# UVA-Computer-Vision-Lab/midvision-probe

Hardware: AMD Instinct MI355X
Metric: images/sec feature-extract+probe-step, ViT-B/16 224^2 (higher is better)
Workload: dtype f16x2 (compensated fp16 pairs of activations and frozen weights, two f16 MFMA products per contraction, fp32 accumulate, feature error as bf16x3; attention: Q.K^T the same two products over compensated pairs, P.V fp16 probabilities x (fp16 + bf16) V; probe, fp32 residual/LN/softmax/loss as in bf16x3

## Files before the change

### include/mvp_hip.h

```cpp
#ifndef MVP_HIP_H
#define MVP_HIP_H

#include <stdint.h>

#ifdef __cplusplus
extern "C" {
#endif

#define MVP_OK 0
#define MVP_EINVAL (-1)
#define MVP_ELAUNCH (-2)
#define MVP_ENODEV (-3)

#define MVP_PREC_BF16 1
#define MVP_PREC_BF16X3 3
#define MVP_PREC_F16X2 2

#define MVP_ACT_NONE 0
#define MVP_ACT_GELU 1
#define MVP_ACT_RELU 2
#define MVP_ACT_QUICK_GELU 3
#define MVP_ACT_GELU_TANH 4

typedef uint16_t mvp_bf16;

typedef struct {
  int abi_version;
  int device_count;
  int gfx950;
  int cu_count;
  char arch[64];
} mvp_info_t;
#define MVP_ABI_VERSION 8
int mvp_get_info(mvp_info_t* out);
const char* mvp_strerror(int code);
int mvp_sizeof(const char* struct_name);

typedef struct {
  const float* src;
  mvp_bf16* hi;
  mvp_bf16* lo;
  int64_t n;
} mvp_split_bf16_args;
int mvp_split_bf16(const mvp_split_bf16_args*, void* stream);

typedef struct {
  const float* images;
  mvp_bf16* out_hi;
  mvp_bf16* out_lo;
  int B, C, H, W;
  int P;
  int gh, gw;
  int pad_top, pad_left;
} mvp_patch_gather_args;
int mvp_patch_gather(const mvp_patch_gather_args*, void* stream);
typedef struct mvp_patch_gather_ld_args mvp_patch_gather_ld_args;
struct mvp_patch_gather_ld_args {
  mvp_patch_gather_args g;
  int ldk;
};
int mvp_patch_gather_ld(const mvp_patch_gather_ld_args*, void* stream);

typedef struct {
  const mvp_bf16* a_hi; const mvp_bf16* a_lo;
  const mvp_bf16* w_hi; const mvp_bf16* w_lo;
  const float* bias;
  const float* residual;
  float* out_f32;
  mvp_bf16* out_hi;
  mvp_bf16* out_lo;
  int M, N, K;
  int lda, ldw, ldr, ldo, ldob;
  int act;
  int precision;
  int row_group, row_group_stride, row_group_off, res_row_mod;
  int conv, cH, cW, cC, cHo, cWo, ckh, ckw, cstride, cpad, cup;
  const mvp_bf16* zero_page;
  const uint8_t* relu_mask; uint8_t* out_mask; int ldm; int mask_mode;
  const float* residual2;
  int act_after_res;
  int splitk; void* splitk_ws; int64_t splitk_ws_bytes;
  const mvp_bf16* residual_hi; const mvp_bf16* residual_lo;
  int tile_policy;
  int pair_layout;
  int out_pair_layout;
  int out_f16_col0;
} mvp_gemm_args;
#define MVP_TILES_ALONE 0
#define MVP_TILES_SHARED 1
#define MVP_TILES_NO_PP 2
#define MVP_TILES_NO_UNI 4
#define MVP_PAIR_SEPARATE 0
#define MVP_PAIR_A_ILV32 1
#define MVP_PAIR_W_ILV32 2
#define MVP_PAIR_ILV32 3
int mvp_gemm_bias_act_res(const mvp_gemm_args*, void* stream);
int mvp_gemm_pp(const mvp_gemm_args*, void* stream);
int64_t mvp_gemm_splitk_workspace_bytes(int M, int N, int splits);
#define MVP_GEMM_ROUTE_PP 1
#define MVP_GEMM_ROUTE_TILE 2
#define MVP_GEMM_ROUTE_SPLITK 3
#define MVP_GEMM_ROUTE_CONV 4
typedef struct mvp_gemm_route_t mvp_gemm_route_t;
struct mvp_gemm_route_t {
  int family;
  int bm, bn, bk;
  int split;
  int nstage, nw, wnw;
};
int mvp_gemm_route(const mvp_gemm_args*, mvp_gemm_route_t* out);
typedef struct mvp_gemm_scaled_args mvp_gemm_scaled_args;
struct mvp_gemm_scaled_args {
  mvp_gemm_args gemm;
  const float* col_scale;
};
int mvp_gemm_scaled(const mvp_gemm_scaled_args*, void* stream);

typedef struct {
  const float* x; const float* gamma; const float* beta;
  mvp_bf16* out_hi; mvp_bf16* out_lo;
  float* out_f32;
  int M, C;
  float eps;
  int out_layout;
  int out_f16;
} mvp_layernorm_args;
int mvp_layernorm_fwd(const mvp_layernorm_args*, void* stream);

typedef struct {
  const mvp_bf16* qkv_hi; const mvp_bf16* qkv_lo;
  mvp_bf16* out_hi; mvp_bf16* out_lo;
  int B, N, H;
  int ld_qkv, ld_out;
  float scale;
  int precision;
  int out_layout;
  int v_format;
  int out_f16;
} mvp_attention_args;
#define MVP_ATT_V_BF16_PAIR 0
#define MVP_ATT_V_F16 1
#define MVP_ATT_V_F16_QK_F16 2
int mvp_attention_fwd(const mvp_attention_args*, void* stream);

typedef struct mvp_attention_bias_args mvp_attention_bias_args;
struct mvp_attention_bias_args {
  mvp_attention_args att;
  const float* bias;
  int64_t bias_head_stride;
  int ld_bias;
};
int mvp_attention_bias_fwd(const mvp_attention_bias_args*, void* stream);

typedef struct mvp_rope2d_qkv_args mvp_rope2d_qkv_args;
struct mvp_rope2d_qkv_args {
  const float* qkv;
  mvp_bf16* out_hi; mvp_bf16* out_lo;
  const float* cos_tab; const float* sin_tab;
  int M, N, H;
  int n_prefix, gh, gw;
  int tab_rows;
  int ld_in, ld_out;
  int precision, v_format;
};
int mvp_rope2d_qkv(const mvp_rope2d_qkv_args*, void* stream);

typedef struct mvp_gather_rows_args mvp_gather_rows_args;
struct mvp_gather_rows_args {
  const mvp_bf16* in_hi; const mvp_bf16* in_lo;
  mvp_bf16* out_hi; mvp_bf16* out_lo;
  const int* idx;
  int rows, rows_in, cols;
  int ld_in, ld_out;
};
int mvp_gather_rows(const mvp_gather_rows_args*, void* stream);

typedef struct mvp_relpos_terms_args mvp_relpos_terms_args;
struct mvp_relpos_terms_args {
  const float* qkv;
  mvp_bf16* out_hi; mvp_bf16* out_lo;
  float* rel;
  const float* rh; const float* rw;
  int64_t rel_bh_stride;
  int M, N, H;
  int Qh, Qw, Kh, Kw;
  int ld_in, ld_out, ld_rel;
  int precision, v_format;
};
int mvp_relpos_terms(const mvp_relpos_terms_args*, void* stream);

typedef struct mvp_attention_relpos_args mvp_attention_relpos_args;
struct mvp_attention_relpos_args {
  mvp_attention_args att;
  const float* rel;
  int64_t rel_bh_stride;
  int ld_rel;
  int Kh, Kw;
};
int mvp_attention_relpos_fwd(const mvp_attention_relpos_args*, void* stream);

typedef struct {
  const float* cls; const float* pos0; float* x; int B, N, C;
} mvp_cls_rows_args;
int mvp_cls_rows(const mvp_cls_rows_args*, void* stream);
typedef struct mvp_prefix_rows_args mvp_prefix_rows_args;
struct mvp_prefix_rows_args {
  const float* cls; const float* pos0; const float* reg; float* x; int B, N, C, R;
};
int mvp_prefix_rows(const mvp_prefix_rows_args*, void* stream);

typedef struct {
  const float* x;
  const float* gamma; const float* beta;
  float* running_mean; float* running_var;
  float* stats;
  float* nchw;
  mvp_bf16* tok_hi; mvp_bf16* tok_lo; int ld_tok; int col_off;
  mvp_bf16* tokT_hi; mvp_bf16* tokT_lo; int ldT;
  void* workspace; int64_t workspace_bytes;
  int B, N, C, hw;
  float eps, momentum;
  int mode;
  float* cls_out;
  int64_t* num_batches_tracked;
  int defer_running;
  int groups;
  int64_t stats_gstride, nchw_gstride, tok_gstride, cls_gstride;
} mvp_bn_tokens_args;
int64_t mvp_bn_tokens_workspace_bytes(int M, int C);
int mvp_bn_tokens_to_nchw_fwd(const mvp_bn_tokens_args*, void* stream);

typedef struct {
  const float* stats;
  float* running_mean; float* running_var;
  int64_t* num_batches_tracked;
  int C; float momentum;
} mvp_bn_running_update_args;
int mvp_bn_running_update(const mvp_bn_running_update_args*, void* stream);
#define MVP_BN_RUNNING_MAX 8
int mvp_bn_running_update_n(const mvp_bn_running_update_args* items, int n, void* stream);

typedef struct {
  const float* nchw;
  mvp_bf16* tok_hi; mvp_bf16* tok_lo; int ld_tok; int col_off;
  mvp_bf16* tokT_hi; mvp_bf16* tokT_lo; int ldT;
  int B, C, hw;
} mvp_pack_nchw_args;
int mvp_pack_nchw_tokens(const mvp_pack_nchw_args*, void* stream);

#define MVP_RESIZE_NEAREST 0
#define MVP_RESIZE_BILINEAR 1
#define MVP_RESIZE_BICUBIC 2
typedef struct {
  const float* src; float* dst;
  int planes, Hi, Wi, Ho, Wo;
  int mode; int align_corners;
  int channels_last; int C;
  float scale_h, scale_w;
} mvp_resize_args;
int mvp_resize_fwd(const mvp_resize_args*, void* stream);
int mvp_resize_bwd(const mvp_resize_args*, void* stream);
int mvp_resize_aa_fwd(const mvp_resize_args*, void* stream);

typedef struct {
  const float* logits; float* depth; float* inv_sum;
  const float* grad_depth; float* grad_logits;
  int64_t P; int K;
  float min_depth, max_depth;
  int kind;
} mvp_depth_predict_args;
int mvp_depth_predict_fwd(const mvp_depth_predict_args*, void* stream);
int mvp_depth_predict_bwd(const mvp_depth_predict_args*, void* stream);

typedef struct {
  const float* pred; float* target; float* loss; float* grad_pred;
  void* workspace; int64_t workspace_bytes;
  int B; int64_t HW;
  float w_sig, w_grad, max_depth, eps, sigma;
} mvp_depth_loss_args;
int64_t mvp_depth_loss_workspace_bytes(int B, int64_t HW);
int mvp_depth_loss_fwd_bwd(const mvp_depth_loss_args*, void* stream);

typedef struct {
  const float* pred; const float* gt; const uint8_t* mask;
  float* loss; float* grad_pred;
  void* workspace; int64_t workspace_bytes;
  int B; int Cp; int64_t HW;
  float eps;
} mvp_angular_loss_args;
int mvp_angular_loss_fwd_bwd(const mvp_angular_loss_args*, void* stream);

typedef struct {
  const float* x; float* out; int M, N, ld;
  int accumulate;
  void* workspace; int64_t workspace_bytes;
} mvp_colsum_args;
int64_t mvp_colsum_workspace_bytes(int M, int N);
int mvp_colsum(const mvp_colsum_args*, void* stream);

typedef struct {
  float* param; const float* grad; float* exp_avg; float* exp_avg_sq;
  const float* hyper; int64_t n;
  float beta1, beta2, eps, weight_decay, grad_scale;
  float lr, bias_c1, bias_c2;
} mvp_adamw_args;
int mvp_adamw_step(const mvp_adamw_args*, void* stream);

typedef struct {
  const float* src_feat; const float* tgt_feat;
  const float* kp_xy;
  int64_t* out_xy; float* out_val;
  float* workspace; int64_t workspace_bytes;
  int C, h, w, K;
  float* heat_out;
} mvp_corr_argmax_args;
int64_t mvp_corr_workspace_bytes(int C, int h, int w, int K);
int mvp_corr_argmax(const mvp_corr_argmax_args*, void* stream);
typedef struct {
  const float* x; int64_t* out_xy; int K, h, w, max_value;
} mvp_argmax_2d_args;
int mvp_argmax_2d(const mvp_argmax_2d_args*, void* stream);

typedef struct mvp_knn_ratio_args mvp_knn_ratio_args;
struct mvp_knn_ratio_args {
  const float* src_feat; const float* tgt_feat;
  const uint8_t* src_valid; const uint8_t* tgt_valid;
  int32_t* nn_idx;
  float* dist;
  float* weight;
  int32_t* n_valid;
  void* workspace; int64_t workspace_bytes;
  int C, N0, N1;
};
int64_t mvp_knn_workspace_bytes(int C, int N0, int N1);
int mvp_knn_ratio(const mvp_knn_ratio_args*, void* stream);

#define MVP_BN_ACT_MAX_C 8
#define MVP_BN_ACT_NONE 0
#define MVP_BN_ACT_SIGMOID 1
#define MVP_BN_ACT_TANH 2
#define MVP_BN_ACT_WORKSPACE_BYTES 98304
typedef struct mvp_bn_act_args mvp_bn_act_args;
struct mvp_bn_act_args {
  const float* x; float* y;
  const float* gamma; const float* beta;
  float* running_mean; float* running_var; int64_t* num_batches_tracked;
  float* stats;
  const float* grad_y; float* grad_x; float* grad_gamma; float* grad_beta;
  void* workspace; int64_t workspace_bytes;
  int B; int64_t HW; int C; int ld;
  int64_t n;
  float eps, momentum;
  int act, training, accumulate;
};
int mvp_bn_act_fwd(const mvp_bn_act_args*, void* stream);
int mvp_bn_act_bwd(const mvp_bn_act_args*, void* stream);

#define MVP_BCE_WORKSPACE_BYTES 8192
typedef struct mvp_bce_loss_args mvp_bce_loss_args;
struct mvp_bce_loss_args {
  const float* pred; const float* target; float* loss; float* grad_pred;
  void* workspace; int64_t workspace_bytes;
  int64_t N;
};
int mvp_bce_loss_fwd_bwd(const mvp_bce_loss_args*, void* stream);

typedef struct mvp_binary_counts_args mvp_binary_counts_args;
struct mvp_binary_counts_args {
  const float* pred; const float* gt; int64_t* counts;
  int G; int64_t n;
  float threshold;
};
int mvp_binary_counts(const mvp_binary_counts_args*, void* stream);

typedef struct {
  const float* w; mvp_bf16* out_hi; mvp_bf16* out_lo;
  int Cout, Cin, kh, kw, mode;
} mvp_conv_weight_pack_args;
int mvp_conv_weight_pack(const mvp_conv_weight_pack_args*, void* stream);

typedef struct {
  const float* src; float* dst_f32; mvp_bf16* dst_hi; mvp_bf16* dst_lo;
  int B, H, W, C, f; int backward;
} mvp_upsample_cl_args;
int mvp_upsample_nearest_cl(const mvp_upsample_cl_args*, void* stream);

typedef struct {
  const float* g; mvp_bf16* out_hi; mvp_bf16* out_lo;
  int B, H, W, C, f;
} mvp_upconv_boxsum_args;
int mvp_upconv3_grad_boxsum(const mvp_upconv_boxsum_args*, void* stream);

typedef struct {
  const float* t; const float* bias; float* out_f32; mvp_bf16* out_hi; mvp_bf16* out_lo; uint8_t* out_mask;
  int B, H, W, C, f, act;
} mvp_upconv_gather_args;
int mvp_upconv3_fwd_gather(const mvp_upconv_gather_args*, void* stream);

typedef struct {
  const mvp_bf16* g_hi; const mvp_bf16* g_lo; const mvp_bf16* x_hi; const mvp_bf16* x_lo;
  float* partial; float* dw; const mvp_bf16* zero_page;
  int64_t M; int Cout, Cin, ldg, ldx;
  int H, W, Ho, Wo, kh, kw, stride, pad, up;
  int splits, accumulate, precision;
} mvp_gemm_tn_args;
typedef struct {
  const float* pred; const float* gt; float* out; float* scale_shift;
  void* workspace; int64_t workspace_bytes; int B; int64_t HW; int scale_invariant;
} mvp_depth_metrics_args;
typedef struct {
  const float* pred; const float* gt; float* out;
  void* workspace; int64_t workspace_bytes; int B; int Cp; int64_t HW; float t1, t2, t3;
} mvp_snorm_metrics_args;
int64_t mvp_metrics_workspace_bytes(int B);
int mvp_depth_metrics(const mvp_depth_metrics_args*, void* stream);
int mvp_snorm_metrics(const mvp_snorm_metrics_args*, void* stream);
typedef struct {
  const float* x; const float* scale_shift; const float* grad_out; float* out;
  int B; int64_t HW; float lo, hi; int clamp; int backward;
} mvp_scale_shift_args;
int mvp_scale_shift(const mvp_scale_shift_args*, void* stream);

typedef struct {
  const float* pred; const float* gt; const int32_t* seg; const float* scale_shift;
  double* level_sums; double* seg_sums;
  void* workspace; int64_t workspace_bytes;
  int B, H, W, Cp, num_levels, num_ids;
  float t1, t2, t3;
} mvp_metrics_breakdown_args;
int64_t mvp_metrics_breakdown_workspace_bytes(int B, int num_levels, int num_ids);
int mvp_metrics_breakdown(const mvp_metrics_breakdown_args*, void* stream);

typedef struct {
  const float* l0; float* depth; float* inv_sum; uint8_t* gate;
  const float* grad_depth; float* grad_l0;
  int B, h, w, K, f;
  float min_depth, max_depth;
} mvp_linear_bins_args;
int mvp_linear_bins_fwd(const mvp_linear_bins_args*, void* stream);
int mvp_linear_bins_bwd(const mvp_linear_bins_args*, void* stream);

typedef struct {
  const float* src; mvp_bf16* out_hi; mvp_bf16* out_lo;
  int B, C, H, W, Ho, Wo, kh, kw, stride, pad, ldk;
} mvp_im2col_args;
int mvp_im2col_nchw(const mvp_im2col_args*, void* stream);

typedef struct {
  const float* src; float* dst_f32; mvp_bf16* dst_hi; mvp_bf16* dst_lo;
  int B, H, W, C, Ho, Wo, k, stride, pad;
} mvp_maxpool_cl_args;
int mvp_maxpool_cl(const mvp_maxpool_cl_args*, void* stream);

typedef struct {
  const float* images; const mvp_bf16* w_hi; const mvp_bf16* w_lo; const float* bias;
  float* out_f32; mvp_bf16* out_hi; mvp_bf16* out_lo;
  int B, H, W, precision;
} mvp_stem_args;
int mvp_stem7x7_pool(const mvp_stem_args*, void* stream);

typedef struct {
  const float* src; const uint8_t* mask; float* dst_f32; mvp_bf16* dst_hi; mvp_bf16* dst_lo;
  int64_t M; int N, lds, ldm, ldo;
  uint8_t* relu_mask_out;
} mvp_mask_split_args;
int mvp_mask_split(const mvp_mask_split_args*, void* stream);

int64_t mvp_gemm_tn_workspace_bytes(int Cout, int Cin, int kh, int kw, int splits);
int mvp_gemm_tn_conv(const mvp_gemm_tn_args*, void* stream);

#ifdef __cplusplus
}
#endif
#endif
```

### midvision-probe_amd/csrc/head.hip

```cpp
#include "mvp_common.h"

namespace {

__device__ __forceinline__ float bin_value(int k, int K, float lo, float hi) {
  const float step = (hi - lo) / (float)(K - 1);
  return (k < K / 2) ? lo + step * (float)k : hi - step * (float)(K - 1 - k);
}

__device__ __forceinline__ void bil_taps(float scale, int o, int in, int& i0, int& i1, float& w0, float& w1) {
  const float s = fmaxf(scale * ((float)o + 0.5f) - 0.5f, 0.f);
  i0 = min((int)s, in - 1);
  i1 = i0 + (i0 < in - 1 ? 1 : 0);
  w1 = s - (float)i0;
  w0 = 1.f - w1;
}

__global__ __launch_bounds__(256) void linear_bins_fwd_kernel(const mvp_linear_bins_args p) {
  const int lane = threadIdx.x & 63;
  const int Ho = p.h * p.f, Wo = p.w * p.f;
  const int64_t px = (int64_t)blockIdx.x * 4 + (threadIdx.x >> 6);
  if (px >= (int64_t)p.B * Ho * Wo) return;
  const int x = (int)(px % Wo);
  const int64_t r = px / Wo;
  const int y = (int)(r % Ho);
  const int64_t b = r / Ho;
  const float sc = 1.0f / (float)p.f;
  int y0, y1, x0, x1;
  float wy0, wy1, wx0, wx1;
  bil_taps(sc, y, p.h, y0, y1, wy0, wy1);
  bil_taps(sc, x, p.w, x0, x1, wx0, wx1);
  const float* base = p.l0 + b * p.h * p.w * p.K;
  const float* r00 = base + ((size_t)y0 * p.w + x0) * p.K;
  const float* r01 = base + ((size_t)y0 * p.w + x1) * p.K;
  const float* r10 = base + ((size_t)y1 * p.w + x0) * p.K;
  const float* r11 = base + ((size_t)y1 * p.w + x1) * p.K;
  const float w00 = wy0 * wx0, w01 = wy0 * wx1, w10 = wy1 * wx0, w11 = wy1 * wx1;
  float s = 0.f, d = 0.f;
  uint8_t* gate = p.gate + px * (p.K >> 3);
  for (int k = lane * 4; k < p.K; k += 256) {
    const float4 a = *(const float4*)(r00 + k), bq = *(const float4*)(r01 + k), c = *(const float4*)(r10 + k), e = *(const float4*)(r11 + k);
    float l[4] = {wy0 * (wx0 * a.x + wx1 * bq.x) + wy1 * (wx0 * c.x + wx1 * e.x), wy0 * (wx0 * a.y + wx1 * bq.y) + wy1 * (wx0 * c.y + wx1 * e.y),
                  wy0 * (wx0 * a.z + wx1 * bq.z) + wy1 * (wx0 * c.z + wx1 * e.z), wy0 * (wx0 * a.w + wx1 * bq.w) + wy1 * (wx0 * c.w + wx1 * e.w)};
    (void)w00; (void)w01; (void)w10; (void)w11;
    unsigned nib = 0;
#pragma unroll
    for (int q = 0; q < 4; ++q) {
      nib |= (l[q] > 0.f ? 1u : 0u) << q;
      const float pq = fmaxf(l[q], 0.f) + 0.1f;
      s += pq;
      d += pq * bin_value(k + q, p.K, p.min_depth, p.max_depth);
    }
    const unsigned other = __shfl_xor(nib, 1, 64);
    if ((lane & 1) == 0) gate[k >> 3] = (uint8_t)(nib | (other << 4));
  }
  s = wave_sum(s);
  d = wave_sum(d);
  if (lane == 0) {
    const float inv = 1.0f / s;
    p.depth[px] = d * inv;
    p.inv_sum[px] = inv;
  }
}

__global__ __launch_bounds__(256) void linear_bins_bwd_kernel(const mvp_linear_bins_args p) {
  const int lane = threadIdx.x & 63;
  const int Ho = p.h * p.f, Wo = p.w * p.f;
  const int64_t tok = (int64_t)blockIdx.x * 4 + (threadIdx.x >> 6);
  if (tok >= (int64_t)p.B * p.h * p.w) return;
  const int tx = (int)(tok % p.w);
  const int64_t r = tok / p.w;
  const int ty = (int)(r % p.h);
  const int64_t b = r / p.h;
  const float sc = 1.0f / (float)p.f;
  const float ff = (float)p.f;
  int ylo = max(0, (int)floorf(ff * ((float)ty - 0.5f) - 0.5f) - 1), yhi = min(Ho - 1, (int)ceilf(ff * ((float)ty + 1.5f) - 0.5f) + 1);
  int xlo = max(0, (int)floorf(ff * ((float)tx - 0.5f) - 0.5f) - 1), xhi = min(Wo - 1, (int)ceilf(ff * ((float)tx + 1.5f) - 0.5f) + 1);
  if (ty == 0) ylo = 0;
  if (ty == p.h - 1) yhi = Ho - 1;
  if (tx == 0) xlo = 0;
  if (tx == p.w - 1) xhi = Wo - 1;
  const int KB = p.K >> 3;
  for (int k = lane * 4; k < p.K; k += 256) {
    float s1[4] = {0.f, 0.f, 0.f, 0.f}, s2[4] = {0.f, 0.f, 0.f, 0.f};
    for (int oy = ylo; oy <= yhi; ++oy) {
      int i0, i1; float w0, w1;
      bil_taps(sc, oy, p.h, i0, i1, w0, w1);
      const float wy = (i0 == ty ? w0 : 0.f) + (i1 == ty ? w1 : 0.f);
      if (wy == 0.f) continue;
      for (int ox = xlo; ox <= xhi; ++ox) {
        bil_taps(sc, ox, p.w, i0, i1, w0, w1);
        const float wx = (i0 == tx ? w0 : 0.f) + (i1 == tx ? w1 : 0.f);
        if (wx == 0.f) continue;
        const int64_t px = (b * Ho + oy) * Wo + ox;
        const float a = wy * wx * p.grad_depth[px] * p.inv_sum[px];
        const float bb = a * p.depth[px];
        const unsigned byte = p.gate[px * KB + (k >> 3)];
        const unsigned nib = (lane & 1) ? (byte >> 4) : (byte & 15u);
#pragma unroll
        for (int q = 0; q < 4; ++q) {
          const float m = (float)((nib >> q) & 1u);
          s1[q] += a * m;
          s2[q] += bb * m;
        }
      }
    }
    float4 o;
    o.x = bin_value(k, p.K, p.min_depth, p.max_depth) * s1[0] - s2[0];
    o.y = bin_value(k + 1, p.K, p.min_depth, p.max_depth) * s1[1] - s2[1];
    o.z = bin_value(k + 2, p.K, p.min_depth, p.max_depth) * s1[2] - s2[2];
    o.w = bin_value(k + 3, p.K, p.min_depth, p.max_depth) * s1[3] - s2[3];
    *(float4*)(p.grad_l0 + tok * p.K + k) = o;
  }
}


__device__ __forceinline__ int bil_cell(float scale, int o, int in) {
  const float s = scale * ((float)o + 0.5f) - 0.5f;
  return (s < 0.f) ? -1 : min((int)s, in - 1);
}

__global__ __launch_bounds__(256) void linear_bins_fwd_cells(const mvp_linear_bins_args p) {
  __shared__ __attribute__((aligned(16))) uint8_t gate_s[4][16][32];
  __shared__ float dep_s[4][16], inv_s[4][16];
  __shared__ int px_s[4][16];
  const int lane = threadIdx.x & 63, wave = threadIdx.x >> 6;
  const int Ho = p.h * p.f, Wo = p.w * p.f;
  const int cells_x = p.w + 1, cells_y = p.h + 1;
  const int64_t cell = (int64_t)blockIdx.x * 4 + wave;
  if (cell >= (int64_t)p.B * cells_y * cells_x) return;
  const int cx = (int)(cell % cells_x) - 1;
  const int64_t r = cell / cells_x;
  const int cy = (int)(r % cells_y) - 1;
  const int64_t b = r / cells_y;
  const float sc = 1.0f / (float)p.f, ff = (float)p.f;
  const int r0 = max(cy, 0), r1 = min(r0 + 1, p.h - 1), c0 = max(cx, 0), c1 = min(c0 + 1, p.w - 1);
  const float* base = p.l0 + b * p.h * p.w * 256;
  const int k = lane * 4;
  const float4 a = *(const float4*)(base + ((size_t)r0 * p.w + c0) * 256 + k);
  const float4 bq = *(const float4*)(base + ((size_t)r0 * p.w + c1) * 256 + k);
  const float4 c = *(const float4*)(base + ((size_t)r1 * p.w + c0) * 256 + k);
  const float4 e = *(const float4*)(base + ((size_t)r1 * p.w + c1) * 256 + k);
  float bins[4];
#pragma unroll
  for (int q = 0; q < 4; ++q) bins[q] = bin_value(k + q, 256, p.min_depth, p.max_depth);
  const int ylo = max(0, (int)floorf(ff * ((float)cy + 0.5f) - 0.5f) - 1), yhi = min(Ho - 1, (int)ceilf(ff * ((float)cy + 1.5f) - 0.5f) + 1);
  const int xlo = max(0, (int)floorf(ff * ((float)cx + 0.5f) - 0.5f) - 1), xhi = min(Wo - 1, (int)ceilf(ff * ((float)cx + 1.5f) - 0.5f) + 1);
  int npix = 0;
  for (int y = ylo; y <= yhi; ++y) {
    if (bil_cell(sc, y, p.h) != cy) continue;
    int y0, y1; float wy0, wy1;
    bil_taps(sc, y, p.h, y0, y1, wy0, wy1);
    for (int x = xlo; x <= xhi; ++x) {
      if (bil_cell(sc, x, p.w) != cx) continue;
      int x0, x1; float wx0, wx1;
      bil_taps(sc, x, p.w, x0, x1, wx0, wx1);
      const float l[4] = {wy0 * (wx0 * a.x + wx1 * bq.x) + wy1 * (wx0 * c.x + wx1 * e.x), wy0 * (wx0 * a.y + wx1 * bq.y) + wy1 * (wx0 * c.y + wx1 * e.y),
                          wy0 * (wx0 * a.z + wx1 * bq.z) + wy1 * (wx0 * c.z + wx1 * e.z), wy0 * (wx0 * a.w + wx1 * bq.w) + wy1 * (wx0 * c.w + wx1 * e.w)};
      float s = 0.f, d = 0.f;
      unsigned nib = 0;
#pragma unroll
      for (int q = 0; q < 4; ++q) {
        nib |= (l[q] > 0.f ? 1u : 0u) << q;
        const float pq = fmaxf(l[q], 0.f) + 0.1f;
        s += pq;
        d += pq * bins[q];
      }
      const unsigned other = __shfl_xor(nib, 1, 64);
      if ((lane & 1) == 0) gate_s[wave][npix][lane >> 1] = (uint8_t)(nib | (other << 4));
      s = wave_sum(s);
      d = wave_sum(d);
      if (lane == 0) {
        const float inv = 1.0f / s;
        dep_s[wave][npix] = d * inv;
        inv_s[wave][npix] = inv;
        px_s[wave][npix] = (int)(((int)b * Ho + y) * Wo + x);
      }
      ++npix;
    }
  }
  __builtin_amdgcn_fence(__ATOMIC_RELEASE, "wavefront");
  __builtin_amdgcn_wave_barrier();
  __builtin_amdgcn_fence(__ATOMIC_ACQUIRE, "wavefront");
  if (lane < npix) {
    const int px = px_s[wave][lane];
    p.depth[px] = dep_s[wave][lane];
    p.inv_sum[px] = inv_s[wave][lane];
  }
  if (lane < 2 * npix) {
    const int pi = lane >> 1, half = lane & 1;
    *(u32x4_t*)(p.gate + (size_t)px_s[wave][pi] * 32 + half * 16) = *(const u32x4_t*)&gate_s[wave][pi][half * 16];
  }
}

__global__ __launch_bounds__(256) void linear_bins_bwd_fast(const mvp_linear_bins_args p) {
  const int lane = threadIdx.x & 63;
  const int Ho = p.h * p.f, Wo = p.w * p.f;
  const int64_t tok = (int64_t)blockIdx.x * 4 + (threadIdx.x >> 6);
  if (tok >= (int64_t)p.B * p.h * p.w) return;
  const int tx = (int)(tok % p.w);
  const int64_t r = tok / p.w;
  const int ty = (int)(r % p.h);
  const int64_t b = r / p.h;
  const float sc = 1.0f / (float)p.f, ff = (float)p.f;
  int ylo = max(0, (int)floorf(ff * ((float)ty - 0.5f) - 0.5f) - 1), yhi = min(Ho - 1, (int)ceilf(ff * ((float)ty + 1.5f) - 0.5f) + 1);
  int xlo = max(0, (int)floorf(ff * ((float)tx - 0.5f) - 0.5f) - 1), xhi = min(Wo - 1, (int)ceilf(ff * ((float)tx + 1.5f) - 0.5f) + 1);
  if (ty == 0) ylo = 0;
  if (ty == p.h - 1) yhi = Ho - 1;
  if (tx == 0) xlo = 0;
  if (tx == p.w - 1) xhi = Wo - 1;
  const int ny = yhi - ylo + 1, nx = xhi - xlo + 1, ncand = ny * nx;
  const int k = lane * 4;
  float s1[4] = {0.f, 0.f, 0.f, 0.f}, s2[4] = {0.f, 0.f, 0.f, 0.f};
  for (int c0 = 0; c0 < ncand; c0 += 64) {
    const int ci = c0 + lane;
    float a_l = 0.f, bb_l = 0.f;
    int px_l = 0;
    if (ci < ncand) {
      const int oy = ylo + ci / nx, ox = xlo + ci % nx;
      int i0, i1; float w0, w1;
      bil_taps(sc, oy, p.h, i0, i1, w0, w1);
      const float wy = (i0 == ty ? w0 : 0.f) + (i1 == ty ? w1 : 0.f);
      bil_taps(sc, ox, p.w, i0, i1, w0, w1);
      const float wx = (i0 == tx ? w0 : 0.f) + (i1 == tx ? w1 : 0.f);
      if (wy != 0.f && wx != 0.f) {
        px_l = (int)(((int)b * Ho + oy) * Wo + ox);
        a_l = wy * wx * p.grad_depth[px_l] * p.inv_sum[px_l];
        bb_l = a_l * p.depth[px_l];
      }
    }
    unsigned long long live = __ballot(a_l != 0.f || bb_l != 0.f);
    while (live) {
      int idx[8];
      unsigned byte[8];
      int n = 0;
#pragma unroll
      for (int u = 0; u < 8; ++u) {
        idx[u] = -1;
        if (live) {
          idx[u] = __builtin_ctzll(live);
          live &= live - 1;
          n = u + 1;
        }
      }
#pragma unroll
      for (int u = 0; u < 8; ++u)
        if (u < n) byte[u] = p.gate[(size_t)__shfl(px_l, idx[u], 64) * 32 + (lane >> 1)];
#pragma unroll
      for (int u = 0; u < 8; ++u) {
        if (u < n) {
          const float av = __shfl(a_l, idx[u], 64), bv = __shfl(bb_l, idx[u], 64);
          const unsigned nib = (lane & 1) ? (byte[u] >> 4) : (byte[u] & 15u);
#pragma unroll
          for (int q = 0; q < 4; ++q) {
            const float m = (float)((nib >> q) & 1u);
            s1[q] += av * m;
            s2[q] += bv * m;
          }
        }
      }
    }
  }
  float4 o;
  o.x = bin_value(k, 256, p.min_depth, p.max_depth) * s1[0] - s2[0];
  o.y = bin_value(k + 1, 256, p.min_depth, p.max_depth) * s1[1] - s2[1];
  o.z = bin_value(k + 2, 256, p.min_depth, p.max_depth) * s1[2] - s2[2];
  o.w = bin_value(k + 3, 256, p.min_depth, p.max_depth) * s1[3] - s2[3];
  *(float4*)(p.grad_l0 + tok * 256 + k) = o;
}

}

extern "C" int mvp_linear_bins_fwd(const mvp_linear_bins_args* a, void* stream) {
  if (!a || !a->l0 || !a->depth || !a->inv_sum || !a->gate) return MVP_EINVAL;
  if (a->B <= 0 || a->h <= 0 || a->w <= 0 || a->f < 1 || a->K < 8 || (a->K & 7)) return MVP_EINVAL;
  const int64_t P = (int64_t)a->B * a->h * a->f * a->w * a->f;
  static const bool generic = getenv("MVP_BINS_GENERIC") != nullptr;
  if (!generic && a->K == 256 && a->f <= 4 && P < ((int64_t)1 << 31)) {
    const int64_t cells = (int64_t)a->B * (a->h + 1) * (a->w + 1);
    hipLaunchKernelGGL(linear_bins_fwd_cells, dim3((unsigned)((cells + 3) / 4)), dim3(256), 0, (hipStream_t)stream, *a);
  } else {
    hipLaunchKernelGGL(linear_bins_fwd_kernel, dim3((unsigned)((P + 3) / 4)), dim3(256), 0, (hipStream_t)stream, *a);
  }
  MVP_LAUNCH_CHECK();
  return MVP_OK;
}

extern "C" int mvp_linear_bins_bwd(const mvp_linear_bins_args* a, void* stream) {
  if (!a || !a->grad_depth || !a->grad_l0 || !a->depth || !a->inv_sum || !a->gate) return MVP_EINVAL;
  if (a->B <= 0 || a->h <= 0 || a->w <= 0 || a->f < 1 || a->K < 8 || (a->K & 7)) return MVP_EINVAL;
  const int64_t T = (int64_t)a->B * a->h * a->w;
  if (a->K == 256 && a->f <= 4 && T * a->f * a->f < ((int64_t)1 << 31))
    hipLaunchKernelGGL(linear_bins_bwd_fast, dim3((unsigned)((T + 3) / 4)), dim3(256), 0, (hipStream_t)stream, *a);
  else
    hipLaunchKernelGGL(linear_bins_bwd_kernel, dim3((unsigned)((T + 3) / 4)), dim3(256), 0, (hipStream_t)stream, *a);
  MVP_LAUNCH_CHECK();
  return MVP_OK;
}
```

### midvision-probe_amd/csrc/info.hip

```cpp
#include <string.h>

#include "mvp_common.h"

extern "C" int mvp_get_info(mvp_info_t* out) {
  if (!out) return MVP_EINVAL;
  memset(out, 0, sizeof(*out));
  out->abi_version = MVP_ABI_VERSION;
  int n = 0;
  if (hipGetDeviceCount(&n) != hipSuccess) n = 0;
  out->device_count = n;
  if (n > 0) {
    hipDeviceProp_t prop;
    if (hipGetDeviceProperties(&prop, 0) == hipSuccess) {
      strncpy(out->arch, prop.gcnArchName, sizeof(out->arch) - 1);
      out->cu_count = prop.multiProcessorCount;
      out->gfx950 = strncmp(prop.gcnArchName, "gfx950", 6) == 0;
    }
  }
  return MVP_OK;
}

extern "C" int mvp_sizeof(const char* name) {
  if (!name) return -1;
#define MVP_SZ(T) if (strcmp(name, #T) == 0) return (int)sizeof(T);
  MVP_SZ(mvp_info_t) MVP_SZ(mvp_split_bf16_args) MVP_SZ(mvp_patch_gather_args) MVP_SZ(mvp_gemm_args) MVP_SZ(mvp_layernorm_args)
  MVP_SZ(mvp_attention_args) MVP_SZ(mvp_cls_rows_args) MVP_SZ(mvp_bn_tokens_args) MVP_SZ(mvp_pack_nchw_args) MVP_SZ(mvp_resize_args)
  MVP_SZ(mvp_depth_predict_args) MVP_SZ(mvp_depth_loss_args) MVP_SZ(mvp_angular_loss_args) MVP_SZ(mvp_colsum_args) MVP_SZ(mvp_adamw_args)
  MVP_SZ(mvp_corr_argmax_args) MVP_SZ(mvp_conv_weight_pack_args) MVP_SZ(mvp_upsample_cl_args) MVP_SZ(mvp_upconv_boxsum_args) MVP_SZ(mvp_upconv_gather_args) MVP_SZ(mvp_gemm_tn_args)
  MVP_SZ(mvp_depth_metrics_args) MVP_SZ(mvp_snorm_metrics_args) MVP_SZ(mvp_linear_bins_args) MVP_SZ(mvp_im2col_args)
  MVP_SZ(mvp_maxpool_cl_args) MVP_SZ(mvp_mask_split_args) MVP_SZ(mvp_metrics_breakdown_args) MVP_SZ(mvp_argmax_2d_args) MVP_SZ(mvp_scale_shift_args) MVP_SZ(mvp_stem_args) MVP_SZ(mvp_bn_running_update_args)
  MVP_SZ(mvp_gemm_scaled_args) MVP_SZ(mvp_patch_gather_ld_args) MVP_SZ(mvp_prefix_rows_args) MVP_SZ(mvp_gemm_route_t) MVP_SZ(mvp_rope2d_qkv_args) MVP_SZ(mvp_attention_bias_args)
  MVP_SZ(mvp_gather_rows_args) MVP_SZ(mvp_relpos_terms_args) MVP_SZ(mvp_attention_relpos_args) MVP_SZ(mvp_knn_ratio_args)
  MVP_SZ(mvp_bn_act_args) MVP_SZ(mvp_bce_loss_args) MVP_SZ(mvp_binary_counts_args)
#undef MVP_SZ
  return -1;
}

extern "C" const char* mvp_strerror(int code) {
  switch (code) {
    case MVP_OK: return "ok";
    case MVP_EINVAL: return "invalid argument (shape, alignment or NULL pointer)";
    case MVP_ELAUNCH: return "HIP kernel launch failed";
    case MVP_ENODEV: return "no gfx950 device";
    default: return "unknown error";
  }
}
```

### midvision-probe_amd/csrc/optim.hip

```cpp
#include "mvp_common.h"

namespace {

__global__ __launch_bounds__(256) void adamw_kernel(const mvp_adamw_args p) {
  const float lr = p.hyper ? p.hyper[0] : p.lr, bc1 = p.hyper ? p.hyper[1] : p.bias_c1, bc2 = p.hyper ? p.hyper[2] : p.bias_c2;
  const float step_size = lr / bc1;
  const float rbc2 = 1.0f / sqrtf(bc2);
  const float decay = 1.0f - lr * p.weight_decay;
  const int64_t n4 = p.n >> 2;
  for (int64_t i = (int64_t)blockIdx.x * 256 + threadIdx.x; i < n4; i += (int64_t)gridDim.x * 256) {
    float4 w = ((float4*)p.param)[i];
    const float4 g4 = ((const float4*)p.grad)[i];
    float4 m = ((float4*)p.exp_avg)[i];
    float4 v = ((float4*)p.exp_avg_sq)[i];
    float* wp = (float*)&w; const float* gp = (const float*)&g4; float* mp = (float*)&m; float* vp = (float*)&v;
#pragma unroll
    for (int e = 0; e < 4; ++e) {
      const float g = gp[e] * p.grad_scale;
      wp[e] *= decay;
      mp[e] = p.beta1 * mp[e] + (1.f - p.beta1) * g;
      vp[e] = p.beta2 * vp[e] + (1.f - p.beta2) * g * g;
      wp[e] -= step_size * mp[e] / (sqrtf(vp[e]) * rbc2 + p.eps);
    }
    ((float4*)p.param)[i] = w;
    ((float4*)p.exp_avg)[i] = m;
    ((float4*)p.exp_avg_sq)[i] = v;
  }
  if (blockIdx.x == 0 && threadIdx.x < (p.n & 3)) {
    const int64_t i = (n4 << 2) + threadIdx.x;
    const float g = p.grad[i] * p.grad_scale;
    float w = p.param[i] * decay;
    const float m = p.beta1 * p.exp_avg[i] + (1.f - p.beta1) * g;
    const float v = p.beta2 * p.exp_avg_sq[i] + (1.f - p.beta2) * g * g;
    w -= step_size * m / (sqrtf(v) * rbc2 + p.eps);
    p.param[i] = w; p.exp_avg[i] = m; p.exp_avg_sq[i] = v;
  }
}

}

extern "C" int mvp_adamw_step(const mvp_adamw_args* a, void* stream) {
  if (!a || !a->param || !a->grad || !a->exp_avg || !a->exp_avg_sq || a->n <= 0) return MVP_EINVAL;
  if (!a->hyper && !(a->bias_c1 > 0.f && a->bias_c2 > 0.f)) return MVP_EINVAL;
  if (((uintptr_t)a->param | (uintptr_t)a->grad | (uintptr_t)a->exp_avg | (uintptr_t)a->exp_avg_sq) & 15) return MVP_EINVAL;
  int64_t g = ((a->n >> 2) + 255) / 256;
  if (g < 1) g = 1;
  if (g > 2048) g = 2048;
  hipLaunchKernelGGL(adamw_kernel, dim3((unsigned)g), dim3(256), 0, (hipStream_t)stream, *a);
  MVP_LAUNCH_CHECK();
  return MVP_OK;
}
```

### midvision-probe_amd/csrc/probe.hip

```cpp
#include "mvp_common.h"

namespace {

__device__ __forceinline__ float bin_value(int k, int K, float lo, float hi) {
  const float step = (hi - lo) / (float)(K - 1);
  return (k < K / 2) ? lo + step * (float)k : hi - step * (float)(K - 1 - k);
}

__global__ __launch_bounds__(256) void depth_bins_fwd(const mvp_depth_predict_args p) {
  const int lane = threadIdx.x & 63;
  const int64_t px = (int64_t)blockIdx.x * 4 + (threadIdx.x >> 6);
  if (px >= p.P) return;
  const float* l = p.logits + px * p.K;
  float s = 0.f, d = 0.f;
  for (int k = lane * 4; k < p.K; k += 256) {
    const float4 v = *(const float4*)(l + k);
    const float a = fmaxf(v.x, 0.f) + 0.1f, b = fmaxf(v.y, 0.f) + 0.1f, c = fmaxf(v.z, 0.f) + 0.1f, e = fmaxf(v.w, 0.f) + 0.1f;
    s += (a + b) + (c + e);
    d += a * bin_value(k, p.K, p.min_depth, p.max_depth) + b * bin_value(k + 1, p.K, p.min_depth, p.max_depth) +
         c * bin_value(k + 2, p.K, p.min_depth, p.max_depth) + e * bin_value(k + 3, p.K, p.min_depth, p.max_depth);
  }
  s = wave_sum(s);
  d = wave_sum(d);
  if (lane == 0) {
    const float inv = 1.0f / s;
    p.depth[px] = d * inv;
    if (p.inv_sum) p.inv_sum[px] = inv;
  }
}

__global__ __launch_bounds__(256) void depth_bins_bwd(const mvp_depth_predict_args p) {
  const int lane = threadIdx.x & 63;
  const int64_t px = (int64_t)blockIdx.x * 4 + (threadIdx.x >> 6);
  if (px >= p.P) return;
  const float* l = p.logits + px * p.K;
  float* g = p.grad_logits + px * p.K;
  const float depth = p.depth[px];
  const float gs = p.grad_depth[px] * p.inv_sum[px];
  for (int k = lane * 4; k < p.K; k += 256) {
    const float4 v = *(const float4*)(l + k);
    float4 o;
    o.x = v.x > 0.f ? gs * (bin_value(k, p.K, p.min_depth, p.max_depth) - depth) : 0.f;
    o.y = v.y > 0.f ? gs * (bin_value(k + 1, p.K, p.min_depth, p.max_depth) - depth) : 0.f;
    o.z = v.z > 0.f ? gs * (bin_value(k + 2, p.K, p.min_depth, p.max_depth) - depth) : 0.f;
    o.w = v.w > 0.f ? gs * (bin_value(k + 3, p.K, p.min_depth, p.max_depth) - depth) : 0.f;
    *(float4*)(g + k) = o;
  }
}

__global__ __launch_bounds__(256) void depth_sigmoid_fwd(const mvp_depth_predict_args p) {
  for (int64_t i = (int64_t)blockIdx.x * 256 + threadIdx.x; i < p.P; i += (int64_t)gridDim.x * 256) {
    const float s = 1.0f / (1.0f + expf(-p.logits[i]));
    p.depth[i] = p.min_depth + s * (p.max_depth - p.min_depth);
  }
}

__global__ __launch_bounds__(256) void depth_sigmoid_bwd(const mvp_depth_predict_args p) {
  for (int64_t i = (int64_t)blockIdx.x * 256 + threadIdx.x; i < p.P; i += (int64_t)gridDim.x * 256) {
    const float s = 1.0f / (1.0f + expf(-p.logits[i]));
    p.grad_logits[i] = p.grad_depth[i] * (p.max_depth - p.min_depth) * s * (1.0f - s);
  }
}

constexpr int CS_CHUNK = 64;

__host__ __device__ inline int cs_chunk_rows(int M) {
  const int r = (M + 255) / 256;
  return r < CS_CHUNK ? CS_CHUNK : ((r + 3) & ~3);
}

__global__ __launch_bounds__(256) void colsum_partial_kernel(const mvp_colsum_args p, float* part, int chunk) {
  __shared__ float red[4][64];
  const int c = blockIdx.x * 64 + (threadIdx.x & 63);
  const int rg = threadIdx.x >> 6;
  const int r0 = blockIdx.y * chunk, r1 = min(p.M, r0 + chunk);
  float s = 0.f;
  if (c < p.N) {
    float s0 = 0.f, s1 = 0.f, s2 = 0.f, s3 = 0.f;
    int r = r0 + rg;
    for (; r + 12 < r1; r += 16) {
      s0 += p.x[(size_t)r * p.ld + c];
      s1 += p.x[(size_t)(r + 4) * p.ld + c];
      s2 += p.x[(size_t)(r + 8) * p.ld + c];
      s3 += p.x[(size_t)(r + 12) * p.ld + c];
    }
    for (; r < r1; r += 4) s0 += p.x[(size_t)r * p.ld + c];
    s = (s0 + s1) + (s2 + s3);
  }
  red[rg][threadIdx.x & 63] = s;
  __syncthreads();
  if (rg == 0 && c < p.N)
    part[(size_t)blockIdx.y * p.N + c] = (red[0][threadIdx.x] + red[1][threadIdx.x]) + (red[2][threadIdx.x] + red[3][threadIdx.x]);
}

__global__ __launch_bounds__(256) void colsum_final_kernel(const mvp_colsum_args p, const float* part, int nchunk) {
  __shared__ float red[4][64];
  const int lc = threadIdx.x & 63, rg = threadIdx.x >> 6;
  const int c = blockIdx.x * 64 + lc;
  float s0 = 0.f, s1 = 0.f, s2 = 0.f, s3 = 0.f;
  if (c < p.N) {
    int k = rg;
    for (; k + 12 < nchunk; k += 16) {
      s0 += part[(size_t)k * p.N + c];
      s1 += part[(size_t)(k + 4) * p.N + c];
      s2 += part[(size_t)(k + 8) * p.N + c];
      s3 += part[(size_t)(k + 12) * p.N + c];
    }
    for (; k < nchunk; k += 4) s0 += part[(size_t)k * p.N + c];
  }
  red[rg][lc] = (s0 + s1) + (s2 + s3);
  __syncthreads();
  if (rg == 0 && c < p.N) {
    const float s = (red[0][lc] + red[1][lc]) + (red[2][lc] + red[3][lc]);
    p.out[c] = p.accumulate ? p.out[c] + s : s;
  }
}

inline int grid_for(int64_t work) {
  int64_t g = (work + 255) / 256;
  return (int)(g < 1 ? 1 : (g > 4096 ? 4096 : g));
}

}

extern "C" int mvp_depth_predict_fwd(const mvp_depth_predict_args* a, void* stream) {
  if (!a || !a->logits || !a->depth || a->P <= 0 || a->K <= 0) return MVP_EINVAL;
  hipStream_t s = (hipStream_t)stream;
  if (a->kind == 0) {
    if ((a->K & 3) || a->K < 2) return MVP_EINVAL;
    hipLaunchKernelGGL(depth_bins_fwd, dim3((unsigned)((a->P + 3) / 4)), dim3(256), 0, s, *a);
  } else {
    if (a->K != 1) return MVP_EINVAL;
    hipLaunchKernelGGL(depth_sigmoid_fwd, dim3(grid_for(a->P)), dim3(256), 0, s, *a);
  }
  MVP_LAUNCH_CHECK();
  return MVP_OK;
}

extern "C" int mvp_depth_predict_bwd(const mvp_depth_predict_args* a, void* stream) {
  if (!a || !a->logits || !a->grad_depth || !a->grad_logits || a->P <= 0 || a->K <= 0) return MVP_EINVAL;
  hipStream_t s = (hipStream_t)stream;
  if (a->kind == 0) {
    if ((a->K & 3) || !a->depth || !a->inv_sum) return MVP_EINVAL;
    hipLaunchKernelGGL(depth_bins_bwd, dim3((unsigned)((a->P + 3) / 4)), dim3(256), 0, s, *a);
  } else {
    if (a->K != 1) return MVP_EINVAL;
    hipLaunchKernelGGL(depth_sigmoid_bwd, dim3(grid_for(a->P)), dim3(256), 0, s, *a);
  }
  MVP_LAUNCH_CHECK();
  return MVP_OK;
}

extern "C" int64_t mvp_colsum_workspace_bytes(int M, int N) {
  const int chunk = cs_chunk_rows(M);
  return (int64_t)((M + chunk - 1) / chunk) * N * 4;
}

extern "C" int mvp_colsum(const mvp_colsum_args* a, void* stream) {
  if (!a || !a->x || !a->out || !a->workspace || a->M <= 0 || a->N <= 0 || a->ld < a->N) return MVP_EINVAL;
  if (a->workspace_bytes < mvp_colsum_workspace_bytes(a->M, a->N)) return MVP_EINVAL;
  const int chunk = cs_chunk_rows(a->M);
  const int nchunk = (a->M + chunk - 1) / chunk;
  hipStream_t s = (hipStream_t)stream;
  hipLaunchKernelGGL(colsum_partial_kernel, dim3((a->N + 63) / 64, nchunk), dim3(256), 0, s, *a, (float*)a->workspace, chunk);
  hipLaunchKernelGGL(colsum_final_kernel, dim3((a->N + 63) / 64), dim3(256), 0, s, *a, (const float*)a->workspace, nchunk);
  MVP_LAUNCH_CHECK();
  return MVP_OK;
}

namespace {
__global__ __launch_bounds__(256) void mask_split_kernel(const mvp_mask_split_args p) {
  const int64_t total = (int64_t)p.M * p.ldo;
  for (int64_t i = (int64_t)blockIdx.x * 256 + threadIdx.x; i < total; i += (int64_t)gridDim.x * 256) {
    const int c = (int)(i % p.ldo);
    const int64_t r = i / p.ldo;
    float v = 0.f;
    if (c < p.N) {
      v = p.src[r * p.lds + c];
      if (p.mask && !p.mask[r * p.ldm + c]) v = 0.f;
      if (p.relu_mask_out) { const bool on = v > 0.f; v = on ? v : 0.f; p.relu_mask_out[r * p.ldm + c] = on; }
      if (p.dst_f32) p.dst_f32[r * p.lds + c] = v;
    }
    uint16_t h, l;
    split_bf16(v, h, l);
    if (p.dst_hi) p.dst_hi[i] = h;
    if (p.dst_lo) p.dst_lo[i] = l;
  }
}

__global__ __launch_bounds__(256) void mask_split_vec4_kernel(const mvp_mask_split_args p) {
  const int q = p.ldo >> 2;
  const int64_t total = (int64_t)p.M * q;
  for (int64_t i = (int64_t)blockIdx.x * 256 + threadIdx.x; i < total; i += (int64_t)gridDim.x * 256) {
    const int64_t r = i / q;
    const int c = (int)(i - r * q) << 2;
    float4 v = make_float4(0.f, 0.f, 0.f, 0.f);
    if (c < p.N) {
      v = *(const float4*)(p.src + r * p.lds + c);
      if (p.mask) {
        const uint32_t m = *(const uint32_t*)(p.mask + r * p.ldm + c);
        if (!(m & 0xffu)) v.x = 0.f;
        if (!(m & 0xff00u)) v.y = 0.f;
        if (!(m & 0xff0000u)) v.z = 0.f;
        if (!(m & 0xff000000u)) v.w = 0.f;
      }
      if (p.relu_mask_out) {
        const uint32_t m = (v.x > 0.f ? 1u : 0u) | (v.y > 0.f ? 0x100u : 0u) | (v.z > 0.f ? 0x10000u : 0u) | (v.w > 0.f ? 0x1000000u : 0u);
        v.x = fmaxf(v.x, 0.f); v.y = fmaxf(v.y, 0.f); v.z = fmaxf(v.z, 0.f); v.w = fmaxf(v.w, 0.f);
        *(uint32_t*)(p.relu_mask_out + r * p.ldm + c) = m;
      }
      if (p.dst_f32) *(float4*)(p.dst_f32 + r * p.lds + c) = v;
    }
    uint32_t h01, l01, h23, l23;
    split2_bf16(v.x, v.y, h01, l01);
    split2_bf16(v.z, v.w, h23, l23);
    const int64_t o = r * p.ldo + c;
    if (p.dst_hi) *(u32x2_t*)(p.dst_hi + o) = u32x2_t{h01, h23};
    if (p.dst_lo) *(u32x2_t*)(p.dst_lo + o) = u32x2_t{l01, l23};
  }
}
}

extern "C" int mvp_mask_split(const mvp_mask_split_args* a, void* stream) {
  if (!a || !a->src || a->M <= 0 || a->N <= 0 || a->ldo < a->N || a->lds < a->N) return MVP_EINVAL;
  const bool vec = !((a->N | a->ldo | a->lds) & 3) && ((!a->mask && !a->relu_mask_out) || !(a->ldm & 3)) &&
                   !(((uintptr_t)a->src | (uintptr_t)a->dst_f32) & 15) && !(((uintptr_t)a->dst_hi | (uintptr_t)a->dst_lo) & 7) &&
                   !(((uintptr_t)a->mask | (uintptr_t)a->relu_mask_out) & 3);
  int64_t g = ((int64_t)a->M * (vec ? a->ldo >> 2 : a->ldo) + 255) / 256;
  if (g > 16384) g = 16384;
  if (vec)
    hipLaunchKernelGGL(mask_split_vec4_kernel, dim3((unsigned)g), dim3(256), 0, (hipStream_t)stream, *a);
  else
    hipLaunchKernelGGL(mask_split_kernel, dim3((unsigned)g), dim3(256), 0, (hipStream_t)stream, *a);
  MVP_LAUNCH_CHECK();
  return MVP_OK;
}
```

### midvision-probe_amd/mvp/functional.py

```python
from __future__ import annotations

from typing import List, Optional, Sequence, Tuple

import torch

from . import lib, ops, pipeline
from .lib import PREC_BF16, PREC_BF16X3
from .vit import PackedFeatures, lookup_pack

_MODES = {"nearest": lib.RESIZE_NEAREST, "bilinear": lib.RESIZE_BILINEAR, "bicubic": lib.RESIZE_BICUBIC}


def _need_cuda(t: torch.Tensor, what: str):
    if not t.is_cuda:
        raise lib.MvpError(f"{what}: the HIP path needs device tensors (there is no CPU fallback)")


class _Interpolate(torch.autograd.Function):
    @staticmethod
    def forward(ctx, x, Ho, Wo, mode, align, sh, sw):
        _need_cuda(x, "interpolate")
        x = x.contiguous().float()
        B, C, Hi, Wi = x.shape
        y = torch.empty(B, C, Ho, Wo, dtype=torch.float32, device=x.device)
        ops.resize(x, y, B * C, Hi, Wi, Ho, Wo, mode, align_corners=align, scale_h=sh, scale_w=sw)
        ctx.cfg = (B, C, Hi, Wi, Ho, Wo, mode, align, sh, sw)
        return y

    @staticmethod
    def backward(ctx, gy):
        B, C, Hi, Wi, Ho, Wo, mode, align, sh, sw = ctx.cfg
        gy = gy.contiguous().float()
        gx = torch.empty(B, C, Hi, Wi, dtype=torch.float32, device=gy.device)
        ops.resize(gy, gx, B * C, Hi, Wi, Ho, Wo, mode, align_corners=align, scale_h=sh, scale_w=sw, backward=True)
        return gx, None, None, None, None, None, None


def interpolate(x: torch.Tensor, size=None, scale_factor=None, mode: str = "nearest", align_corners: Optional[bool] = None) -> torch.Tensor:
    if mode not in _MODES:
        raise NotImplementedError(f"interpolate mode {mode!r}")
    Hi, Wi = x.shape[-2:]
    sh = sw = 0.0
    if size is not None:
        Ho, Wo = (size, size) if isinstance(size, int) else tuple(int(s) for s in size)
    else:
        sf = (scale_factor, scale_factor) if not isinstance(scale_factor, (tuple, list)) else scale_factor
        sh, sw = float(sf[0]), float(sf[1])
        Ho, Wo = int(Hi * sh), int(Wi * sw)
    return _Interpolate.apply(x, Ho, Wo, _MODES[mode], bool(align_corners), sh, sw)


def resize_antialias(x: torch.Tensor, size) -> torch.Tensor:
    _need_cuda(x, "resize_antialias")
    if x.requires_grad:
        raise lib.MvpError("resize_antialias is forward-only (input side of the frozen backbone)")
    x = x.contiguous().float()
    B, C, Hi, Wi = x.shape
    Ho, Wo = (size, size) if isinstance(size, int) else tuple(int(v) for v in size)
    y = torch.empty(B, C, Ho, Wo, dtype=torch.float32, device=x.device)
    a = lib.ResizeArgs(lib.ptr(x), lib.ptr(y), B * C, Hi, Wi, Ho, Wo, lib.RESIZE_BILINEAR, 0, 0, 0, 0.0, 0.0)
    lib.call("mvp_resize_aa_fwd", a)
    return y


def pack_features(feats: Sequence[torch.Tensor], precision: int) -> PackedFeatures:
    pack = lookup_pack(feats)
    if pack is not None and pack.precision == precision:
        return pack
    B, _, h, w = feats[0].shape
    for f in feats:
        _need_cuda(f, "probe features")
        if f.shape[0] != B or f.shape[-2:] != (h, w):
            raise lib.MvpError("linear head: all feature maps must share batch and resolution (reference quirk Q7)")
    Ctot = sum(int(f.shape[1]) for f in feats)
    pack = PackedFeatures(B, h, w, Ctot, precision, feats[0].device)
    off = 0
    for f in feats:
        C = int(f.shape[1])
        ops.pack_nchw_tokens(f.contiguous().float(), B, C, h * w, tok=pack.tok, ld_tok=pack.Cpad, col_off=off)
        off += C
    return pack


def _grad_dst(param, shape):
    from .optim import grad_destination

    d = grad_destination(param) if param is not None else None
    return d.view(shape) if d is not None and d.numel() == int(torch.Size(shape).numel()) else None


def _head_weight_grad(gl0: torch.Tensor, K: int, pack: PackedFeatures, pr: int, dst: Optional[torch.Tensor] = None) -> torch.Tensor:
    from . import conv
    dev = gl0.device
    Kg = (K + 127) // 128 * 128
    if Kg != K:
        gpad = gl0.new_zeros(pack.M, Kg)
        gpad[:, :K] = gl0
        gl0 = gpad
    gp = ops.split_bf16(gl0, pr)
    dW = dst if (dst is not None and pack.Cpad == pack.Ctot and tuple(dst.shape) == (K, pack.Cpad)) else torch.empty(K, pack.Cpad, dtype=torch.float32, device=dev)
    geo = dict(B=pack.B, H=pack.h, W=pack.w, C=pack.Cpad, Ho=pack.h, Wo=pack.w, kh=1, kw=1, stride=1, pad=0, up=0)
    conv.conv_dw(gp, Kg, pack.tok, pack.Cpad, geo, K, dW, precision=pr)
    return dW[:, :pack.Ctot]


class _LinearHeadK1(torch.autograd.Function):

    @staticmethod
    def forward(ctx, weight, bias, pack: PackedFeatures, precision: int):
        K, Ctot = weight.shape[0], pack.Ctot
        K4 = (K + 3) // 4 * 4
        dev = weight.device
        w2 = weight.detach().reshape(K, Ctot).float()
        b1 = bias.detach().float()
        if K4 != K or pack.Cpad != Ctot:
            wpad = w2.new_zeros(K4, pack.Cpad)
            wpad[:K, :Ctot] = w2
            w2 = wpad
            b1 = torch.cat([b1, b1.new_zeros(K4 - K)], 0)
        wp = ops.split_bf16(w2.contiguous(), precision)
        l0 = torch.empty(pack.M, K4, dtype=torch.float32, device=dev)
        ops.gemm(pack.tok, wp, pack.M, K4, pack.Cpad, bias=b1.contiguous(), out_f32=l0, precision=precision)
        B, h, w = pack.B, pack.h, pack.w
        lq = torch.empty(B, 4 * h, 4 * w, K4, dtype=torch.float32, device=dev)
        ops.resize(l0, lq, B, h, w, 4 * h, 4 * w, lib.RESIZE_BILINEAR, channels_last=True, Cdim=K4, scale_h=4.0, scale_w=4.0)
        ctx.pack, ctx.precision, ctx.K, ctx.K4 = pack, precision, K, K4
        ctx.wshape = weight.shape
        ctx.generation = pack.generation
        return lq

    @staticmethod
    def backward(ctx, glq):
        pack, pr, K, K4 = ctx.pack, ctx.precision, ctx.K, ctx.K4
        B, h, w, Ctot = pack.B, pack.h, pack.w, pack.Ctot
        dev = glq.device
        if pack.generation != ctx.generation:
            raise lib.MvpError("linear head backward: the backbone ran again before this backward and overwrote the packed "
                               "features of this step (call backward before the next model(images))")
        glq = glq.contiguous()
        gl0 = torch.empty(pack.M, K4, dtype=torch.float32, device=dev)
        ops.resize(glq, gl0, B, h, w, 4 * h, 4 * w, lib.RESIZE_BILINEAR, channels_last=True, Cdim=K4, scale_h=4.0, scale_w=4.0, backward=True)
        dW = _head_weight_grad(gl0, K4, pack, pr)
        db = torch.empty(K4, dtype=torch.float32, device=dev)
        ops.colsum(gl0, db, pack.M, K4)
        return dW[:K].reshape(ctx.wshape), db[:K], None, None


def linear_head_k1(feats: Sequence[torch.Tensor], weight: torch.Tensor, bias: torch.Tensor, precision: int) -> torch.Tensor:
    pack = pack_features(list(feats), precision)
    return _LinearHeadK1.apply(weight, bias, pack, precision)


def linear_bins_forward(weight, bias, pack: PackedFeatures, precision: int, min_depth: float, max_depth: float):
    K, Ctot = weight.shape[0], pack.Ctot
    dev = weight.device
    w2 = weight.detach().reshape(K, Ctot).float()
    if pack.Cpad != Ctot:
        wpad = w2.new_zeros(K, pack.Cpad)
        wpad[:, :Ctot] = w2
        w2 = wpad
    wp = ops.split_bf16(w2.contiguous(), precision)
    l0 = torch.empty(pack.M, K, dtype=torch.float32, device=dev)
    ops.gemm(pack.tok, wp, pack.M, K, pack.Cpad, bias=bias.detach().float().contiguous(), out_f32=l0, precision=precision)
    B, h, w = pack.B, pack.h, pack.w
    P = B * 16 * h * w
    depth = torch.empty(B, 1, 4 * h, 4 * w, dtype=torch.float32, device=dev)
    inv = torch.empty(P, dtype=torch.float32, device=dev)
    gate = torch.empty(P, K // 8, dtype=torch.uint8, device=dev)
    a = lib.LinearBinsArgs(lib.ptr(l0), lib.ptr(depth), lib.ptr(inv), lib.ptr(gate), None, None, B, h, w, K, 4, min_depth, max_depth)
    lib.call("mvp_linear_bins_fwd", a)
    return depth, inv, gate


def linear_bins_backward(gd, depth, inv, gate, pack: PackedFeatures, precision: int, K: int, min_depth: float, max_depth: float,
                         dw_dst: Optional[torch.Tensor], db_dst: Optional[torch.Tensor]):
    B, h, w = pack.B, pack.h, pack.w
    dev = gd.device
    gl0 = torch.empty(pack.M, K, dtype=torch.float32, device=dev)
    a = lib.LinearBinsArgs(None, lib.ptr(depth), lib.ptr(inv), lib.ptr(gate), lib.ptr(gd.contiguous().float()), lib.ptr(gl0), B, h, w, K, 4,
                           min_depth, max_depth)
    lib.call("mvp_linear_bins_bwd", a)
    dW = _head_weight_grad(gl0, K, pack, precision, dst=dw_dst)
    db = db_dst
    if db is None:
        db = torch.empty(K, dtype=torch.float32, device=dev)
    ops.colsum(gl0, db, pack.M, K)
    return dW, db


class _LinearBinsHead(torch.autograd.Function):

    @staticmethod
    def forward(ctx, weight, bias, pack: PackedFeatures, precision: int, n_bins: int, min_depth: float, max_depth: float):
        depth, inv, gate = linear_bins_forward(weight, bias, pack, precision, min_depth, max_depth)
        ctx.pack, ctx.precision, ctx.cfg = pack, precision, (weight.shape[0], min_depth, max_depth)
        ctx.wshape, ctx.generation = weight.shape, pack.generation
        ctx.params = (weight, bias)
        ctx.save_for_backward(depth, inv, gate)
        return depth

    @staticmethod
    def backward(ctx, gd):
        depth, inv, gate = ctx.saved_tensors
        pack, pr = ctx.pack, ctx.precision
        K, mn, mx = ctx.cfg
        if pack.generation != ctx.generation:
            raise lib.MvpError("linear head backward: the backbone ran again before this backward and overwrote the packed "
                               "features of this step (call backward before the next model(images))")
        wparam, bparam = ctx.params
        dW, db = linear_bins_backward(gd, depth, inv, gate, pack, pr, K, mn, mx, _grad_dst(wparam, (K, pack.Ctot)), _grad_dst(bparam, (K,)))
        return dW.reshape(ctx.wshape), db, None, None, None, None, None


def linear_bins_head(feats: Sequence[torch.Tensor], weight, bias, precision: int, n_bins: int, min_depth: float, max_depth: float) -> torch.Tensor:
    pack = pack_features(list(feats), precision)
    return _LinearBinsHead.apply(weight, bias, pack, precision, n_bins, float(min_depth), float(max_depth))


class _LinearHeadKxK(torch.autograd.Function):

    @staticmethod
    def forward(ctx, weight, bias, feats, precision):
        from . import conv as cv

        B, _, h, w = feats[0].shape
        dev = weight.device
        K, Ctot, k, _ = weight.shape
        Cp = (Ctot + 127) // 128 * 128
        H4, W4 = 4 * h, 4 * w
        M = B * H4 * W4
        up = ops.empty_pair((M, Cp), precision, dev)
        wsrc = weight.detach()
        if Cp != Ctot:
            for t in up:
                if t is not None:
                    t.zero_()
            wsrc = wsrc.new_zeros(K, Cp, k, k)
            wsrc[:, :Ctot] = weight.detach()
        off = 0
        for f in feats:
            C = int(f.shape[1])
            big = torch.empty(B, C, H4, W4, dtype=torch.float32, device=dev)
            ops.resize(f.contiguous().float(), big, B * C, h, w, H4, W4, lib.RESIZE_BILINEAR, scale_h=4.0, scale_w=4.0)
            ops.pack_nchw_tokens(big, B, C, H4 * W4, tok=up, ld_tok=Cp, col_off=off)
            off += C
        K4 = (K + 3) // 4 * 4
        g = cv.geom(B, H4, W4, Cp, k, k, 1, k // 2)
        b4 = torch.cat([bias.detach().float(), bias.new_zeros(K4 - K).float()]) if K4 != K else bias.detach().float().contiguous()
        lq = torch.empty(B, H4, W4, K4, dtype=torch.float32, device=dev)
        cv.conv_gemm(up, g, cv.pack_weight(wsrc, 0, precision, pad_cout_to=K4), K4, bias=b4, out_f32=lq, precision=precision)
        ctx.up, ctx.g, ctx.cfg = up, g, (K, K4, M, precision)
        ctx.wshape = weight.shape
        return lq

    @staticmethod
    def backward(ctx, glq):
        from . import conv as cv

        K, K4, M, pr = ctx.cfg
        dev = glq.device
        gl = glq.contiguous().float().reshape(M, K4)
        LG = (K4 + 127) // 128 * 128
        gP = cv.mask_split(gl, None, M, K4, ldo=LG, precision=pr)
        Cp, Ctot = ctx.g["C"], ctx.wshape[1]
        dW = torch.empty((ctx.wshape[0], Cp) + tuple(ctx.wshape[2:]), dtype=torch.float32, device=dev)
        cv.conv_dw(gP, LG, ctx.up, Cp, ctx.g, K, dW, precision=pr)
        if Cp != Ctot:
            dW = dW[:, :Ctot].contiguous()
        db = torch.empty(K4, dtype=torch.float32, device=dev)
        ops.colsum(gl, db, M, K4)
        return dW, db[:K].contiguous(), None, None


def linear_head_kxk(feats: Sequence[torch.Tensor], weight: torch.Tensor, bias: torch.Tensor, precision: int) -> torch.Tensor:
    for f in feats:
        _need_cuda(f, "probe features")
    return _LinearHeadKxK.apply(weight, bias, list(feats), precision)


class _ConvValid(torch.autograd.Function):

    @staticmethod
    def forward(ctx, x, weight, bias, precision, need_dx):
        from . import conv as cv

        _need_cuda(x, "conv2d_valid")
        B, C, H, W = x.shape
        Cout, Cin, k, k2 = weight.shape
        if Cin != C or k != k2 or H < k or W < k:
            raise lib.MvpError(f"conv2d_valid: input {tuple(x.shape)} does not fit a {tuple(weight.shape)} kernel")
        if C % 128:
            raise lib.MvpError(f"conv2d_valid on the HIP path needs input channels % 128 == 0 (got {C})")
        dev = x.device
        tok = ops.empty_pair((B * H * W, C), precision, dev)
        ops.pack_nchw_tokens(x.contiguous().float(), B, C, H * W, tok=tok, ld_tok=C, col_off=0)
        g = cv.geom(B, H, W, C, k, k, 1, 0)
        N4 = (Cout + 3) // 4 * 4
        b4 = bias.detach().float().contiguous()
        if N4 != Cout:
            b4 = torch.cat([b4, b4.new_zeros(N4 - Cout)])
        y = torch.empty(B, g["Ho"], g["Wo"], N4, dtype=torch.float32, device=dev)
        cv.conv_gemm(tok, g, cv.pack_weight(weight, 0, precision, pad_cout_to=N4), N4, bias=b4, out_f32=y, precision=precision)
        ctx.tok, ctx.g, ctx.cfg = tok, g, (Cout, N4, precision, bool(need_dx))
        ctx.save_for_backward(weight)
        return y[..., :Cout].permute(0, 3, 1, 2)

    @staticmethod
    def backward(ctx, gy):
        from . import conv as cv

        (weight,) = ctx.saved_tensors
        Cout, N4, pr, need_dx = ctx.cfg
        g = ctx.g
        B, H, W, C, Ho, Wo, k = g["B"], g["H"], g["W"], g["C"], g["Ho"], g["Wo"], g["kh"]
        dev = gy.device
        M = B * Ho * Wo
        gl = torch.zeros(M, N4, dtype=torch.float32, device=dev)
        gl[:, :Cout] = gy.permute(0, 2, 3, 1).reshape(M, Cout)
        LG = (N4 + 127) // 128 * 128
        gP = cv.mask_split(gl, None, M, N4, ldo=LG, precision=pr)
        dW = torch.empty(weight.shape, dtype=torch.float32, device=dev)
        cv.conv_dw(gP, LG, ctx.tok, C, g, Cout, dW, precision=pr)
        db = torch.empty(N4, dtype=torch.float32, device=dev)
        ops.colsum(gl, db, M, N4)
        dx = None
        if need_dx:
            wT = cv.pack_weight(weight, 1, pr, pad_cout_to=LG)
            dxc = torch.empty(B, H, W, C, dtype=torch.float32, device=dev)
            cv.conv_gemm(gP, cv.geom(B, Ho, Wo, LG, k, k, 1, k - 1), wT, C, out_f32=dxc, precision=pr)
            dx = dxc.permute(0, 3, 1, 2)
        return dx, dW, db[:Cout].contiguous(), None, None


def conv2d_valid(x: torch.Tensor, weight: torch.Tensor, bias: torch.Tensor, precision: int, need_input_grad: bool = True) -> torch.Tensor:
    return _ConvValid.apply(x, weight, bias, precision, need_input_grad)


class _DepthPredict(torch.autograd.Function):
    @staticmethod
    def forward(ctx, logits_cl, K, min_depth, max_depth, kind):
        B, H, W, Kp = logits_cl.shape
        if Kp != K and not (kind == 1 and K == 1):
            raise lib.MvpError("depth predictor: channel padding is only supported for sigmoid heads")
        P = B * H * W
        lg = logits_cl.contiguous()
        if kind == 1 and Kp != 1:
            lg = lg[..., :1].contiguous()
        depth = torch.empty(B, 1, H, W, dtype=torch.float32, device=lg.device)
        inv = torch.empty(P, dtype=torch.float32, device=lg.device) if kind == 0 else None
        ops.depth_predict_fwd(lg, depth, inv, P, K, min_depth, max_depth, kind)
        ctx.save_for_backward(lg, depth, inv if inv is not None else depth)
        ctx.cfg = (P, K, Kp, min_depth, max_depth, kind, logits_cl.shape)
        return depth

    @staticmethod
    def backward(ctx, gd):
        lg, depth, inv = ctx.saved_tensors
        P, K, Kp, mn, mx, kind, shape = ctx.cfg
        gl = torch.empty_like(lg)
        ops.depth_predict_bwd(lg, depth, inv if kind == 0 else None, gd.contiguous().float(), gl, P, K, mn, mx, kind)
        if kind == 1 and Kp != 1:
            full = gl.new_zeros(shape)
            full[..., :1] = gl
            gl = full
        return gl, None, None, None, None


def depth_bins(logits_cl, n_bins, min_depth, max_depth):
    return _DepthPredict.apply(logits_cl, n_bins, float(min_depth), float(max_depth), 0)


def depth_sigmoid(logits_cl, min_depth, max_depth):
    return _DepthPredict.apply(logits_cl, 1, float(min_depth), float(max_depth), 1)


_ONE = {}


def _one(dev) -> torch.Tensor:
    t = _ONE.get(dev)
    if t is None:
        t = _ONE[dev] = torch.ones((), dtype=torch.float32, device=dev)
        pipeline.publish()
    return t


def backward(loss: torch.Tensor) -> None:
    torch.autograd.backward(loss, grad_tensors=_one(loss.device))


def _scaled(grad: torch.Tensor, g: torch.Tensor) -> torch.Tensor:
    one = _ONE.get(g.device)
    if one is not None and g.data_ptr() == one.data_ptr():
        return grad
    return grad * g


class _DepthLoss(torch.autograd.Function):
    @staticmethod
    def forward(ctx, pred, target, w_sig, w_grad, max_depth):
        _need_cuda(pred, "DepthLoss")
        if not (target.is_cuda and target.is_contiguous() and target.dtype == torch.float32):
            raise lib.MvpError("DepthLoss: target must be a contiguous fp32 device tensor (it is modified in place, quirk Q2)")
        B = pred.shape[0]
        HW = pred.numel() // B
        p = pred.contiguous().float()
        out = torch.empty(4, dtype=torch.float32, device=p.device)
        grad = torch.empty_like(p)
        ws = torch.empty(ops.depth_loss_workspace_bytes(B, HW) // 4 + 4, dtype=torch.float32, device=p.device)
        ops.depth_loss(p, target, out, grad, ws, B, HW, w_sig, w_grad, max_depth)
        ctx.save_for_backward(grad)
        ctx.parts = out
        return out[0]

    @staticmethod
    def backward(ctx, g):
        (grad,) = ctx.saved_tensors
        return _scaled(grad, g), None, None, None, None


def depth_loss(pred, target, w_sig=10.0, w_grad=0.5, max_depth=10.0):
    return _DepthLoss.apply(pred, target, float(w_sig), float(w_grad), float(max_depth))


class _AngularLoss(torch.autograd.Function):
    @staticmethod
    def forward(ctx, pred, gt, mask, eps):
        _need_cuda(pred, "angular_loss")
        B, Cp = pred.shape[:2]
        HW = pred.numel() // (B * Cp)
        p = pred.contiguous().float()
        m = mask.reshape(B, -1).to(torch.uint8).contiguous()
        out = torch.empty(4, dtype=torch.float32, device=p.device)
        grad = torch.empty_like(p)
        ws = torch.empty(1024, dtype=torch.float32, device=p.device)
        ops.angular_loss(p, gt.contiguous().float(), m, out, grad, ws, B, Cp, HW, eps)
        ctx.save_for_backward(grad)
        return out[0]

    @staticmethod
    def backward(ctx, g):
        (grad,) = ctx.saved_tensors
        return _scaled(grad, g), None, None, None


def angular_loss(pred, gt, mask, uncertainty_aware=False, eps=1e-4):
    assert mask.ndim == 4, f"mask should be (batch x height x width) not {mask.shape}"
    assert pred.shape[1] == (4 if uncertainty_aware else 3)
    return _AngularLoss.apply(pred, gt, mask, float(eps))


_BN_ACTS = {"none": lib.BN_ACT_NONE, "sigmoid": lib.BN_ACT_SIGMOID, "tanh": lib.BN_ACT_TANH}


def _rows_view(x: torch.Tensor):
    B, Cdim, H, W = x.shape
    sb, sc, sh, sw = x.stride()
    ld = sw
    if x.dtype == torch.float32 and (sc == 1 or Cdim == 1) and ld >= Cdim and sh == W * ld and sb == H * W * ld:
        return x, ld
    return x.permute(0, 2, 3, 1).contiguous().float(), Cdim


class _BnAct(torch.autograd.Function):
    @staticmethod
    def forward(ctx, x, gamma, beta, bn, act, training, n_factor):
        _need_cuda(x, "bn_act")
        B, Cdim, H, W = x.shape
        HW = H * W
        xr, ld = _rows_view(x)
        dev = x.device
        y = torch.empty(B, Cdim, H, W, dtype=torch.float32, device=dev)
        stats = ws = None
        kw = {}
        if act == lib.BN_ACT_SIGMOID:
            stats = torch.empty(3 * Cdim, dtype=torch.float32, device=dev)
            ws = ops.bn_act_workspace(dev)
            kw = dict(gamma=gamma.detach(), beta=beta.detach(), stats=stats, workspace=ws, n=n_factor * B * HW, eps=float(bn.eps),
                      momentum=float(bn.momentum), running_mean=bn.running_mean, running_var=bn.running_var,
                      num_batches_tracked=bn.num_batches_tracked if training else None)
        ops.bn_act_fwd(xr, y, B, HW, Cdim, ld, act, training, **kw)
        ctx.save_for_backward(xr, stats if stats is not None else y)
        ctx.cfg = (B, Cdim, H, W, ld, act, training, tuple(x.shape), tuple(x.stride()))
        ctx.params = (gamma, beta)
        ctx.ws = ws
        return y

    @staticmethod
    def backward(ctx, gy):
        xr, stats = ctx.saved_tensors
        B, Cdim, H, W, ld, act, training, shape, stride = ctx.cfg
        gamma, beta = ctx.params
        dev = gy.device
        gy = gy.contiguous().float()
        gx = torch.empty(B, H, W, ld, dtype=torch.float32, device=dev)
        dg = db = None
        kw = {}
        if act == lib.BN_ACT_SIGMOID:
            dg, db = _grad_dst(gamma, (Cdim,)), _grad_dst(beta, (Cdim,))
            dg = dg if dg is not None else torch.empty(Cdim, dtype=torch.float32, device=dev)
            db = db if db is not None else torch.empty(Cdim, dtype=torch.float32, device=dev)
            kw = dict(gamma=gamma.detach(), beta=beta.detach(), stats=stats, workspace=ctx.ws, grad_gamma=dg, grad_beta=db)
        ops.bn_act_bwd(xr, gy, gx, B, H * W, Cdim, ld, act, training, **kw)
        return gx[..., :Cdim].permute(0, 3, 1, 2), dg, db, None, None, None, None


def bn_act(x: torch.Tensor, bn=None, act: str = "sigmoid", training: bool = True, n_factor: int = 1) -> torch.Tensor:
    a = _BN_ACTS[act]
    if a == lib.BN_ACT_SIGMOID:
        if bn is None or not bn.affine or not bn.track_running_stats or bn.momentum is None:
            raise lib.MvpError("bn_act: the sigmoid form needs an affine nn.BatchNorm2d with running statistics and a fixed momentum")
        return _BnAct.apply(x, bn.weight, bn.bias, bn, a, bool(training), int(n_factor))
    return _BnAct.apply(x, None, None, None, a, False, 1)


class _BceLoss(torch.autograd.Function):
    @staticmethod
    def forward(ctx, pred, target):
        _need_cuda(pred, "bce_loss")
        if tuple(pred.shape) != tuple(target.shape):
            raise ValueError(f"bce_loss: prediction {tuple(pred.shape)} and target {tuple(target.shape)} differ (nn.BCELoss does not broadcast)")
        p = pred.contiguous().float()
        t = target.contiguous().float()
        out = torch.empty(1, dtype=torch.float32, device=p.device)
        grad = torch.empty_like(p)
        ws = torch.empty(lib.BCE_WORKSPACE_BYTES // 8, dtype=torch.float64, device=p.device)
        ops.bce_loss(p, t, out, grad, ws, p.numel())
        ctx.save_for_backward(grad)
        return out[0]

    @staticmethod
    def backward(ctx, g):
        (grad,) = ctx.saved_tensors
        return _scaled(grad, g), None


def bce_loss(pred, target):
    return _BceLoss.apply(pred, target)
```

### midvision-probe_amd/mvp/lib.py

```python
from __future__ import annotations

import ctypes as C
import os
from typing import Optional

import torch

_HERE = os.path.dirname(os.path.abspath(__file__))
LIB_PATH = os.environ.get("MVP_LIB") or os.path.join(os.path.dirname(_HERE), "csrc", "libmvp_hip.so")

PREC_BF16 = 1
PREC_BF16X3 = 3
PREC_F16X2 = 2
ACT_NONE, ACT_GELU, ACT_RELU, ACT_QUICK_GELU, ACT_GELU_TANH = 0, 1, 2, 3, 4
RESIZE_NEAREST, RESIZE_BILINEAR, RESIZE_BICUBIC = 0, 1, 2
PAIR_SEPARATE, PAIR_A_ILV32, PAIR_W_ILV32 = 0, 1, 2
BN_ACT_NONE, BN_ACT_SIGMOID, BN_ACT_TANH = 0, 1, 2
BN_ACT_WORKSPACE_BYTES, BCE_WORKSPACE_BYTES = 98304, 8192
BN_RUNNING_MAX = 8
TILES_SHARED, TILES_NO_PP, TILES_NO_UNI = 1, 2, 4
ROUTE_PP, ROUTE_TILE, ROUTE_SPLITK, ROUTE_CONV = 1, 2, 3, 4

_vp = C.c_void_p
_i = C.c_int
_f = C.c_float
_i64 = C.c_int64


class MvpError(RuntimeError):
    pass


class Info(C.Structure):
    _fields_ = [("abi_version", _i), ("device_count", _i), ("gfx950", _i), ("cu_count", _i), ("arch", C.c_char * 64)]


class SplitArgs(C.Structure):
    _fields_ = [("src", _vp), ("hi", _vp), ("lo", _vp), ("n", _i64)]


class PatchGatherArgs(C.Structure):
    _fields_ = [("images", _vp), ("out_hi", _vp), ("out_lo", _vp), ("B", _i), ("C", _i), ("H", _i), ("W", _i),
                ("P", _i), ("gh", _i), ("gw", _i), ("pad_top", _i), ("pad_left", _i)]


class GemmArgs(C.Structure):
    _fields_ = [("a_hi", _vp), ("a_lo", _vp), ("w_hi", _vp), ("w_lo", _vp), ("bias", _vp), ("residual", _vp),
                ("out_f32", _vp), ("out_hi", _vp), ("out_lo", _vp), ("M", _i), ("N", _i), ("K", _i),
                ("lda", _i), ("ldw", _i), ("ldr", _i), ("ldo", _i), ("ldob", _i), ("act", _i), ("precision", _i),
                ("row_group", _i), ("row_group_stride", _i), ("row_group_off", _i), ("res_row_mod", _i),
                ("conv", _i), ("cH", _i), ("cW", _i), ("cC", _i), ("cHo", _i), ("cWo", _i), ("ckh", _i), ("ckw", _i),
                ("cstride", _i), ("cpad", _i), ("cup", _i), ("zero_page", _vp), ("relu_mask", _vp), ("out_mask", _vp), ("ldm", _i), ("mask_mode", _i),
                ("residual2", _vp), ("act_after_res", _i), ("splitk", _i), ("splitk_ws", _vp), ("splitk_ws_bytes", _i64),
                ("residual_hi", _vp), ("residual_lo", _vp), ("tile_policy", _i), ("pair_layout", _i), ("out_pair_layout", _i),
                ("out_f16_col0", _i)]


class LayerNormArgs(C.Structure):
    _fields_ = [("x", _vp), ("gamma", _vp), ("beta", _vp), ("out_hi", _vp), ("out_lo", _vp), ("out_f32", _vp),
                ("M", _i), ("C", _i), ("eps", _f), ("out_layout", _i), ("out_f16", _i)]


class AttentionArgs(C.Structure):
    _fields_ = [("qkv_hi", _vp), ("qkv_lo", _vp), ("out_hi", _vp), ("out_lo", _vp), ("B", _i), ("N", _i), ("H", _i),
                ("ld_qkv", _i), ("ld_out", _i), ("scale", _f), ("precision", _i), ("out_layout", _i), ("v_format", _i), ("out_f16", _i)]


class AttentionBiasArgs(C.Structure):
    _fields_ = [("att", AttentionArgs), ("bias", _vp), ("bias_head_stride", _i64), ("ld_bias", _i)]


class GatherRowsArgs(C.Structure):
    _fields_ = [("in_hi", _vp), ("in_lo", _vp), ("out_hi", _vp), ("out_lo", _vp), ("idx", _vp), ("rows", _i), ("rows_in", _i), ("cols", _i),
                ("ld_in", _i), ("ld_out", _i)]


class RelposTermsArgs(C.Structure):
    _fields_ = [("qkv", _vp), ("out_hi", _vp), ("out_lo", _vp), ("rel", _vp), ("rh", _vp), ("rw", _vp), ("rel_bh_stride", _i64),
                ("M", _i), ("N", _i), ("H", _i), ("Qh", _i), ("Qw", _i), ("Kh", _i), ("Kw", _i), ("ld_in", _i), ("ld_out", _i), ("ld_rel", _i),
                ("precision", _i), ("v_format", _i)]


class AttentionRelposArgs(C.Structure):
    _fields_ = [("att", AttentionArgs), ("rel", _vp), ("rel_bh_stride", _i64), ("ld_rel", _i), ("Kh", _i), ("Kw", _i)]


class ClsRowsArgs(C.Structure):
    _fields_ = [("cls", _vp), ("pos0", _vp), ("x", _vp), ("B", _i), ("N", _i), ("C", _i)]


class GemmScaledArgs(C.Structure):
    _fields_ = [("gemm", GemmArgs), ("col_scale", _vp)]


class GemmRoute(C.Structure):
    _fields_ = [("family", _i), ("bm", _i), ("bn", _i), ("bk", _i), ("split", _i), ("nstage", _i), ("nw", _i), ("wnw", _i)]


class PatchGatherLdArgs(C.Structure):
    _fields_ = [("g", PatchGatherArgs), ("ldk", _i)]


class PrefixRowsArgs(C.Structure):
    _fields_ = [("cls", _vp), ("pos0", _vp), ("reg", _vp), ("x", _vp), ("B", _i), ("N", _i), ("C", _i), ("R", _i)]


class Rope2dQkvArgs(C.Structure):
    _fields_ = [("qkv", _vp), ("out_hi", _vp), ("out_lo", _vp), ("cos_tab", _vp), ("sin_tab", _vp), ("M", _i), ("N", _i), ("H", _i),
                ("n_prefix", _i), ("gh", _i), ("gw", _i), ("tab_rows", _i), ("ld_in", _i), ("ld_out", _i), ("precision", _i), ("v_format", _i)]


class BnTokensArgs(C.Structure):
    _fields_ = [("x", _vp), ("gamma", _vp), ("beta", _vp), ("running_mean", _vp), ("running_var", _vp), ("stats", _vp),
                ("nchw", _vp), ("tok_hi", _vp), ("tok_lo", _vp), ("ld_tok", _i), ("col_off", _i),
                ("tokT_hi", _vp), ("tokT_lo", _vp), ("ldT", _i),
                ("workspace", _vp), ("workspace_bytes", _i64),
                ("B", _i), ("N", _i), ("C", _i), ("hw", _i), ("eps", _f), ("momentum", _f), ("mode", _i), ("cls_out", _vp), ("num_batches_tracked", _vp),
                ("defer_running", _i), ("groups", _i), ("stats_gstride", _i64), ("nchw_gstride", _i64), ("tok_gstride", _i64), ("cls_gstride", _i64)]


class BnRunningUpdateArgs(C.Structure):
    _fields_ = [("stats", _vp), ("running_mean", _vp), ("running_var", _vp), ("num_batches_tracked", _vp), ("C", _i), ("momentum", _f)]


class PackNchwArgs(C.Structure):
    _fields_ = [("nchw", _vp), ("tok_hi", _vp), ("tok_lo", _vp), ("ld_tok", _i), ("col_off", _i),
                ("tokT_hi", _vp), ("tokT_lo", _vp), ("ldT", _i), ("B", _i), ("C", _i), ("hw", _i)]


class ResizeArgs(C.Structure):
    _fields_ = [("src", _vp), ("dst", _vp), ("planes", _i), ("Hi", _i), ("Wi", _i), ("Ho", _i), ("Wo", _i),
                ("mode", _i), ("align_corners", _i), ("channels_last", _i), ("C", _i), ("scale_h", _f), ("scale_w", _f)]


class DepthPredictArgs(C.Structure):
    _fields_ = [("logits", _vp), ("depth", _vp), ("inv_sum", _vp), ("grad_depth", _vp), ("grad_logits", _vp),
                ("P", _i64), ("K", _i), ("min_depth", _f), ("max_depth", _f), ("kind", _i)]


class DepthLossArgs(C.Structure):
    _fields_ = [("pred", _vp), ("target", _vp), ("loss", _vp), ("grad_pred", _vp), ("workspace", _vp),
                ("workspace_bytes", _i64), ("B", _i), ("HW", _i64), ("w_sig", _f), ("w_grad", _f), ("max_depth", _f),
                ("eps", _f), ("sigma", _f)]


class AngularLossArgs(C.Structure):
    _fields_ = [("pred", _vp), ("gt", _vp), ("mask", _vp), ("loss", _vp), ("grad_pred", _vp), ("workspace", _vp),
                ("workspace_bytes", _i64), ("B", _i), ("Cp", _i), ("HW", _i64), ("eps", _f)]


class ColsumArgs(C.Structure):
    _fields_ = [("x", _vp), ("out", _vp), ("M", _i), ("N", _i), ("ld", _i), ("accumulate", _i), ("workspace", _vp), ("workspace_bytes", _i64)]


class AdamWArgs(C.Structure):
    _fields_ = [("param", _vp), ("grad", _vp), ("exp_avg", _vp), ("exp_avg_sq", _vp), ("hyper", _vp), ("n", _i64),
                ("beta1", _f), ("beta2", _f), ("eps", _f), ("weight_decay", _f), ("grad_scale", _f),
                ("lr", _f), ("bias_c1", _f), ("bias_c2", _f)]


class CorrArgmaxArgs(C.Structure):
    _fields_ = [("src_feat", _vp), ("tgt_feat", _vp), ("kp_xy", _vp), ("out_xy", _vp), ("out_val", _vp),
                ("workspace", _vp), ("workspace_bytes", _i64), ("C", _i), ("h", _i), ("w", _i), ("K", _i), ("heat_out", _vp)]


class Argmax2dArgs(C.Structure):
    _fields_ = [("x", _vp), ("out_xy", _vp), ("K", _i), ("h", _i), ("w", _i), ("max_value", _i)]


class KnnRatioArgs(C.Structure):
    _fields_ = [("src_feat", _vp), ("tgt_feat", _vp), ("src_valid", _vp), ("tgt_valid", _vp), ("nn_idx", _vp), ("dist", _vp), ("weight", _vp),
                ("n_valid", _vp), ("workspace", _vp), ("workspace_bytes", _i64), ("C", _i), ("N0", _i), ("N1", _i)]


class BnActArgs(C.Structure):
    _fields_ = [("x", _vp), ("y", _vp), ("gamma", _vp), ("beta", _vp), ("running_mean", _vp), ("running_var", _vp), ("num_batches_tracked", _vp),
                ("stats", _vp), ("grad_y", _vp), ("grad_x", _vp), ("grad_gamma", _vp), ("grad_beta", _vp), ("workspace", _vp), ("workspace_bytes", _i64),
                ("B", _i), ("HW", _i64), ("C", _i), ("ld", _i), ("n", _i64), ("eps", _f), ("momentum", _f), ("act", _i), ("training", _i), ("accumulate", _i)]


class BceLossArgs(C.Structure):
    _fields_ = [("pred", _vp), ("target", _vp), ("loss", _vp), ("grad_pred", _vp), ("workspace", _vp), ("workspace_bytes", _i64), ("N", _i64)]


class BinaryCountsArgs(C.Structure):
    _fields_ = [("pred", _vp), ("gt", _vp), ("counts", _vp), ("G", _i), ("n", _i64), ("threshold", _f)]


class ScaleShiftArgs(C.Structure):
    _fields_ = [("x", _vp), ("scale_shift", _vp), ("grad_out", _vp), ("out", _vp), ("B", _i), ("HW", _i64), ("lo", _f), ("hi", _f),
                ("clamp", _i), ("backward", _i)]


class MetricsBreakdownArgs(C.Structure):
    _fields_ = [("pred", _vp), ("gt", _vp), ("seg", _vp), ("scale_shift", _vp), ("level_sums", _vp), ("seg_sums", _vp),
                ("workspace", _vp), ("workspace_bytes", _i64), ("B", _i), ("H", _i), ("W", _i), ("Cp", _i), ("num_levels", _i), ("num_ids", _i),
                ("t1", _f), ("t2", _f), ("t3", _f)]


class ConvWeightPackArgs(C.Structure):
    _fields_ = [("w", _vp), ("out_hi", _vp), ("out_lo", _vp), ("Cout", _i), ("Cin", _i), ("kh", _i), ("kw", _i), ("mode", _i)]


class UpsampleClArgs(C.Structure):
    _fields_ = [("src", _vp), ("dst_f32", _vp), ("dst_hi", _vp), ("dst_lo", _vp), ("B", _i), ("H", _i), ("W", _i), ("C", _i),
                ("f", _i), ("backward", _i)]


class UpconvBoxsumArgs(C.Structure):
    _fields_ = [("g", _vp), ("out_hi", _vp), ("out_lo", _vp), ("B", _i), ("H", _i), ("W", _i), ("C", _i), ("f", _i)]


class UpconvGatherArgs(C.Structure):
    _fields_ = [("t", _vp), ("bias", _vp), ("out_f32", _vp), ("out_hi", _vp), ("out_lo", _vp), ("out_mask", _vp),
                ("B", _i), ("H", _i), ("W", _i), ("C", _i), ("f", _i), ("act", _i)]


class DepthMetricsArgs(C.Structure):
    _fields_ = [("pred", _vp), ("gt", _vp), ("out", _vp), ("scale_shift", _vp), ("workspace", _vp), ("workspace_bytes", _i64),
                ("B", _i), ("HW", _i64), ("scale_invariant", _i)]


class SnormMetricsArgs(C.Structure):
    _fields_ = [("pred", _vp), ("gt", _vp), ("out", _vp), ("workspace", _vp), ("workspace_bytes", _i64), ("B", _i), ("Cp", _i),
                ("HW", _i64), ("t1", _f), ("t2", _f), ("t3", _f)]


class LinearBinsArgs(C.Structure):
    _fields_ = [("l0", _vp), ("depth", _vp), ("inv_sum", _vp), ("gate", _vp), ("grad_depth", _vp), ("grad_l0", _vp),
                ("B", _i), ("h", _i), ("w", _i), ("K", _i), ("f", _i), ("min_depth", _f), ("max_depth", _f)]


class Im2colArgs(C.Structure):
    _fields_ = [("src", _vp), ("out_hi", _vp), ("out_lo", _vp), ("B", _i), ("C", _i), ("H", _i), ("W", _i), ("Ho", _i), ("Wo", _i),
                ("kh", _i), ("kw", _i), ("stride", _i), ("pad", _i), ("ldk", _i)]


class MaxpoolClArgs(C.Structure):
    _fields_ = [("src", _vp), ("dst_f32", _vp), ("dst_hi", _vp), ("dst_lo", _vp), ("B", _i), ("H", _i), ("W", _i), ("C", _i),
                ("Ho", _i), ("Wo", _i), ("k", _i), ("stride", _i), ("pad", _i)]


class StemArgs(C.Structure):
    _fields_ = [("images", _vp), ("w_hi", _vp), ("w_lo", _vp), ("bias", _vp), ("out_f32", _vp), ("out_hi", _vp), ("out_lo", _vp),
                ("B", _i), ("H", _i), ("W", _i), ("precision", _i)]


class MaskSplitArgs(C.Structure):
    _fields_ = [("src", _vp), ("mask", _vp), ("dst_f32", _vp), ("dst_hi", _vp), ("dst_lo", _vp), ("M", _i64), ("N", _i),
                ("lds", _i), ("ldm", _i), ("ldo", _i), ("relu_mask_out", _vp)]


class GemmTnArgs(C.Structure):
    _fields_ = [("g_hi", _vp), ("g_lo", _vp), ("x_hi", _vp), ("x_lo", _vp), ("partial", _vp), ("dw", _vp), ("zero_page", _vp),
                ("M", _i64), ("Cout", _i), ("Cin", _i), ("ldg", _i), ("ldx", _i), ("H", _i), ("W", _i), ("Ho", _i), ("Wo", _i),
                ("kh", _i), ("kw", _i), ("stride", _i), ("pad", _i), ("up", _i), ("splits", _i), ("accumulate", _i), ("precision", _i)]


SYMBOLS = {
    "mvp_get_info": None,
    "mvp_strerror": None,
    "mvp_sizeof": None,
    "mvp_split_bf16": SplitArgs,
    "mvp_patch_gather": PatchGatherArgs,
    "mvp_gemm_bias_act_res": GemmArgs,
    "mvp_gemm_splitk_workspace_bytes": None,
    "mvp_gemm_route": None,
    "mvp_layernorm_fwd": LayerNormArgs,
    "mvp_attention_fwd": AttentionArgs,
    "mvp_cls_rows": ClsRowsArgs,
    "mvp_bn_tokens_workspace_bytes": None,
    "mvp_bn_tokens_to_nchw_fwd": BnTokensArgs,
    "mvp_bn_running_update": BnRunningUpdateArgs,
    "mvp_bn_running_update_n": None,
    "mvp_pack_nchw_tokens": PackNchwArgs,
    "mvp_resize_fwd": ResizeArgs,
    "mvp_resize_bwd": ResizeArgs,
    "mvp_resize_aa_fwd": ResizeArgs,
    "mvp_depth_predict_fwd": DepthPredictArgs,
    "mvp_depth_predict_bwd": DepthPredictArgs,
    "mvp_depth_loss_workspace_bytes": None,
    "mvp_depth_loss_fwd_bwd": DepthLossArgs,
    "mvp_angular_loss_fwd_bwd": AngularLossArgs,
    "mvp_colsum_workspace_bytes": None,
    "mvp_colsum": ColsumArgs,
    "mvp_adamw_step": AdamWArgs,
    "mvp_corr_argmax": CorrArgmaxArgs,
    "mvp_corr_workspace_bytes": None,
    "mvp_argmax_2d": Argmax2dArgs,
    "mvp_scale_shift": ScaleShiftArgs,
    "mvp_metrics_breakdown_workspace_bytes": None,
    "mvp_metrics_breakdown": MetricsBreakdownArgs,
    "mvp_conv_weight_pack": ConvWeightPackArgs,
    "mvp_upsample_nearest_cl": UpsampleClArgs,
    "mvp_upconv3_grad_boxsum": UpconvBoxsumArgs,
    "mvp_upconv3_fwd_gather": UpconvGatherArgs,
    "mvp_mask_split": MaskSplitArgs,
    "mvp_metrics_workspace_bytes": None,
    "mvp_depth_metrics": DepthMetricsArgs,
    "mvp_snorm_metrics": SnormMetricsArgs,
    "mvp_linear_bins_fwd": LinearBinsArgs,
    "mvp_linear_bins_bwd": LinearBinsArgs,
    "mvp_im2col_nchw": Im2colArgs,
    "mvp_maxpool_cl": MaxpoolClArgs,
    "mvp_stem7x7_pool": StemArgs,
    "mvp_gemm_pp": GemmArgs,
    "mvp_gemm_tn_workspace_bytes": None,
    "mvp_gemm_tn_conv": GemmTnArgs,
    "mvp_gemm_scaled": GemmScaledArgs,
    "mvp_patch_gather_ld": PatchGatherLdArgs,
    "mvp_prefix_rows": PrefixRowsArgs,
    "mvp_rope2d_qkv": Rope2dQkvArgs,
    "mvp_attention_bias_fwd": AttentionBiasArgs,
    "mvp_gather_rows": GatherRowsArgs,
    "mvp_relpos_terms": RelposTermsArgs,
    "mvp_attention_relpos_fwd": AttentionRelposArgs,
    "mvp_knn_ratio": KnnRatioArgs,
    "mvp_knn_workspace_bytes": None,
    "mvp_bn_act_fwd": BnActArgs,
    "mvp_bn_act_bwd": BnActArgs,
    "mvp_bce_loss_fwd_bwd": BceLossArgs,
    "mvp_binary_counts": BinaryCountsArgs,
}

NEW_STRUCTS_ABI7 = {"mvp_gemm_scaled_args": GemmScaledArgs, "mvp_patch_gather_ld_args": PatchGatherLdArgs, "mvp_prefix_rows_args": PrefixRowsArgs}

NEW_STRUCTS_ABI8 = {"mvp_gemm_route_t": GemmRoute, "mvp_rope2d_qkv_args": Rope2dQkvArgs, "mvp_attention_bias_args": AttentionBiasArgs,
                    "mvp_gather_rows_args": GatherRowsArgs, "mvp_relpos_terms_args": RelposTermsArgs,
                    "mvp_attention_relpos_args": AttentionRelposArgs, "mvp_knn_ratio_args": KnnRatioArgs,
                    "mvp_bn_act_args": BnActArgs, "mvp_bce_loss_args": BceLossArgs,
                    "mvp_binary_counts_args": BinaryCountsArgs}

_lib: Optional[C.CDLL] = None


def load() -> C.CDLL:
    global _lib
    if _lib is not None:
        return _lib
    if not os.path.exists(LIB_PATH):
        raise MvpError(
            f"{LIB_PATH} not found: the HIP extension is not built. Run `python -c 'import __graft_entry__ as g; g.build()'` "
            "(or `make -C midvision-probe_amd/csrc`). There is no CPU fallback for the product path."
        )
    lib = C.CDLL(LIB_PATH)
    for name, st in SYMBOLS.items():
        fn = getattr(lib, name)
        if st is not None:
            fn.argtypes = [C.POINTER(st), _vp]
            fn.restype = _i
    lib.mvp_bn_running_update_n.argtypes = [C.POINTER(BnRunningUpdateArgs), _i, _vp]
    lib.mvp_bn_running_update_n.restype = _i
    lib.mvp_get_info.argtypes = [C.POINTER(Info)]
    lib.mvp_get_info.restype = _i
    lib.mvp_strerror.argtypes = [_i]
    lib.mvp_strerror.restype = C.c_char_p
    lib.mvp_corr_workspace_bytes.argtypes = [_i, _i, _i, _i]
    lib.mvp_corr_workspace_bytes.restype = _i64
    lib.mvp_knn_workspace_bytes.argtypes = [_i, _i, _i]
    lib.mvp_knn_workspace_bytes.restype = _i64
    lib.mvp_sizeof.argtypes = [C.c_char_p]
    lib.mvp_sizeof.restype = _i
    lib.mvp_bn_tokens_workspace_bytes.argtypes = [_i, _i]
    lib.mvp_bn_tokens_workspace_bytes.restype = _i64
    lib.mvp_colsum_workspace_bytes.argtypes = [_i, _i]
    lib.mvp_colsum_workspace_bytes.restype = _i64
    lib.mvp_metrics_breakdown_workspace_bytes.argtypes = [_i, _i, _i]
    lib.mvp_metrics_breakdown_workspace_bytes.restype = _i64
    lib.mvp_metrics_workspace_bytes.argtypes = [_i]
    lib.mvp_metrics_workspace_bytes.restype = _i64
    lib.mvp_gemm_route.argtypes = [C.POINTER(GemmArgs), C.POINTER(GemmRoute)]
    lib.mvp_gemm_route.restype = _i
    lib.mvp_gemm_splitk_workspace_bytes.argtypes = [_i, _i, _i]
    lib.mvp_gemm_splitk_workspace_bytes.restype = _i64
    lib.mvp_gemm_tn_workspace_bytes.argtypes = [_i, _i, _i, _i, _i]
    lib.mvp_gemm_tn_workspace_bytes.restype = _i64
    lib.mvp_depth_loss_workspace_bytes.argtypes = [_i, _i64]
    lib.mvp_depth_loss_workspace_bytes.restype = _i64
    _lib = lib
    return lib


def info() -> Info:
    out = Info()
    check(load().mvp_get_info(C.byref(out)), "mvp_get_info")
    return out


def check(code: int, what: str) -> None:
    if code != 0:
        raise MvpError(f"{what} failed: {load().mvp_strerror(code).decode()} (code {code})")


_raw_stream = getattr(torch._C, "_cuda_getCurrentRawStream", None)
_cur_device = getattr(torch._C, "_cuda_getDevice", None)


def stream_ptr() -> int:
    if _raw_stream is not None and _cur_device is not None:
        return _raw_stream(_cur_device())
    return torch.cuda.current_stream().cuda_stream


def ptr(t: Optional[torch.Tensor]) -> Optional[int]:
    if t is None:
        return None
    if not t.is_cuda:
        raise MvpError("expected a device tensor (the HIP path has no CPU fallback)")
    return t.data_ptr()


TRACE_CALLS = None


def call(name: str, args: C.Structure) -> None:
    if TRACE_CALLS is None:
        check(getattr(load(), name)(C.byref(args), stream_ptr()), name)
        return
    e0, e1 = torch.cuda.Event(enable_timing=True), torch.cuda.Event(enable_timing=True)
    e0.record()
    check(getattr(load(), name)(C.byref(args), stream_ptr()), name)
    e1.record()
    TRACE_CALLS.append((name, stream_ptr(), e0, e1))
```

### midvision-probe_amd/mvp/ops.py

```python
from __future__ import annotations

import ctypes
import functools
from typing import Optional, Tuple

import torch

from . import lib, pipeline
from .lib import PREC_BF16, PREC_BF16X3

Pair = Tuple[torch.Tensor, Optional[torch.Tensor]]


class IlvPair:

    def __init__(self, rows: int, cols: int, device):
        if cols % 32:
            raise lib.MvpError("an interleaved pair needs cols % 32 == 0")
        self.rows, self.cols = rows, cols
        self.t = torch.empty(rows, 2 * cols, dtype=torch.bfloat16, device=device)

    def separate(self) -> Pair:
        v = self.t.view(self.rows, self.cols // 32, 2, 32)
        return v[:, :, 0].reshape(self.rows, self.cols).contiguous(), v[:, :, 1].reshape(self.rows, self.cols).contiguous()

_TRACE = None


def set_trace(lst) -> None:
    global _TRACE
    _TRACE = lst


def _traced(kind: str, tile: str, precision: int, work: float, fn) -> None:
    if _TRACE is None:
        fn()
        return
    e0, e1 = torch.cuda.Event(enable_timing=True), torch.cuda.Event(enable_timing=True)
    e0.record()
    fn()
    e1.record()
    _TRACE.append((kind, tile, precision, work, e0, e1))


@functools.lru_cache(maxsize=None)
def _route_label(M: int, N: int, K: int, precision: int, splitk: int, tile_policy: int, a_ilv: bool = False, ext: bool = False) -> str:
    a = lib.GemmArgs(a_hi=16, a_lo=16, w_hi=16, w_lo=16, out_f32=16, out_hi=16, out_lo=16, M=M, N=N, K=K, lda=2 * K if a_ilv else K, ldw=K,
                     ldr=N, ldo=N, ldob=N, precision=precision, splitk=splitk, tile_policy=tile_policy,
                     pair_layout=lib.PAIR_A_ILV32 if a_ilv else lib.PAIR_SEPARATE, out_mask=16 if ext else None, ldm=N)
    r = lib.GemmRoute()
    if lib.load().mvp_gemm_route(ctypes.byref(a), ctypes.byref(r)) != 0:
        return ""
    if r.family == lib.ROUTE_PP:
        return f"pp {r.bm}, {r.bn}, {r.bk}, {r.split}"
    return f"{r.bm}, {r.bn}, {r.bk}, {r.split}, {r.nstage}" + (", splitk" if r.family == lib.ROUTE_SPLITK else "")


def gemm_tile(M: int, N: int, K: int = 0, precision: int = PREC_BF16X3, splitk: int = 1, tile_policy: int = 0) -> str:
    label = _route_label(M, N, K, precision, splitk, tile_policy)
    if not label:
        raise lib.MvpError(f"mvp_gemm_route: no kernel takes M={M} N={N} K={K} precision={precision} splitk={splitk}")
    return label


def _chk(t: torch.Tensor, dtype, name: str):
    if t.dtype != dtype or not t.is_cuda or not t.is_contiguous():
        raise lib.MvpError(f"{name}: expected contiguous {dtype} device tensor, got {t.dtype} {t.device} contiguous={t.is_contiguous()}")


def empty_pair(shape, precision: int, device) -> Pair:
    hi = torch.empty(shape, dtype=torch.bfloat16, device=device)
    lo = torch.empty(shape, dtype=torch.bfloat16, device=device) if precision == PREC_BF16X3 else None
    return hi, lo


def zeros_pair(shape, precision: int, device) -> Pair:
    hi = torch.zeros(shape, dtype=torch.bfloat16, device=device)
    lo = torch.zeros(shape, dtype=torch.bfloat16, device=device) if precision == PREC_BF16X3 else None
    return hi, lo


def split_bf16(src: torch.Tensor, precision: int = PREC_BF16X3) -> Pair:
    src = src.contiguous()
    _chk(src, torch.float32, "split_bf16.src")
    hi, lo = empty_pair(src.shape, precision, src.device)
    a = lib.SplitArgs(lib.ptr(src), lib.ptr(hi), lib.ptr(lo), src.numel())
    lib.call("mvp_split_bf16", a)
    return hi, lo


F16X2_S = 2.0 ** -6


def f16x2_weight(w: torch.Tensor) -> Pair:
    w = w.detach().double().contiguous()
    t = (1.0 - F16X2_S) * w
    hi = t.clamp(-65504.0, 65504.0).to(torch.float16)
    lo = ((w + (t - hi.double()) / F16X2_S) / 8.0).clamp(-65504.0, 65504.0).to(torch.float16)
    return hi.view(torch.bfloat16).contiguous(), lo.view(torch.bfloat16).contiguous()


def split_f16_comp(src: torch.Tensor) -> Pair:
    x = src.float()
    hi = x.clamp(-65504.0, 65504.0).half()
    h = hi.float()
    lo = ((x - h) * 8.0 + h * 0.125).clamp(-65504.0, 65504.0).half()
    return hi.view(torch.bfloat16).contiguous(), lo.view(torch.bfloat16).contiguous()


def split_f16_bf16(src: torch.Tensor) -> Pair:
    x = src.float()
    hi = x.clamp(-65504.0, 65504.0).half()
    return hi.view(torch.bfloat16).contiguous(), (x - hi.float()).bfloat16().contiguous()


def interleave_pair(pair: Pair) -> Optional[torch.Tensor]:
    hi, lo = pair
    if lo is None or hi.dim() != 2 or hi.shape[1] % 32:
        return None
    R, K = hi.shape
    return torch.stack((hi.view(R, K // 32, 32), lo.view(R, K // 32, 32)), dim=2).reshape(R, 2 * K).contiguous()


def patch_gather(images: torch.Tensor, out: Pair, P: int, gh: int, gw: int, pad_top: int, pad_left: int) -> None:
    _chk(images, torch.float32, "patch_gather.images")
    B, Cc, H, W = images.shape
    a = lib.PatchGatherArgs(lib.ptr(images), lib.ptr(out[0]), lib.ptr(out[1]), B, Cc, H, W, P, gh, gw, pad_top, pad_left)
    lib.call("mvp_patch_gather", a)


def patch_gather_ld(images: torch.Tensor, out: Pair, P: int, gh: int, gw: int, pad_top: int, pad_left: int, ldk: int) -> None:
    _chk(images, torch.float32, "patch_gather_ld.images")
    B, Cc, H, W = images.shape
    g = lib.PatchGatherArgs(lib.ptr(images), lib.ptr(out[0]), lib.ptr(out[1]), B, Cc, H, W, P, gh, gw, pad_top, pad_left)
    lib.call("mvp_patch_gather_ld", lib.PatchGatherLdArgs(g, int(ldk)))


_SPLITK_WS = {}


def splitk_auto(M: int, N: int, K: int) -> int:
    if N <= 256 and K >= 2048 and ((M + 127) // 128) * ((N + 63) // 64) <= 128:
        return 4
    return 1


def _ws_key(device):
    if pipeline.pipelined():
        return (device, "slot", pipeline.current_slot())
    return (device, lib.stream_ptr())


def _splitk_workspace(M: int, N: int, S: int, device) -> torch.Tensor:
    need = int(lib.load().mvp_gemm_splitk_workspace_bytes(M, N, S))
    key = _ws_key(device)
    ws = _SPLITK_WS.get(key)
    if ws is None or ws.numel() < need:
        ws = _SPLITK_WS[key] = torch.zeros(max(need, 32 << 20), dtype=torch.uint8, device=device)
    return ws


def gemm(a: Pair, w: Pair, M: int, N: int, K: int, *, bias=None, residual=None, out_f32=None, out: Optional[Pair] = None,
         act: int = lib.ACT_NONE, precision: int = PREC_BF16X3, lda=None, ldw=None, ldr=None, ldo=None, ldob=None,
         row_group=0, row_group_stride=0, row_group_off=0, res_row_mod=0, act_after_res=False, out_mask=None, ldm=0,
         splitk: Optional[int] = None, residual_pair: Optional[Pair] = None,
         w_ilv: Optional[torch.Tensor] = None, f16_col0: int = 0, col_scale: Optional[torch.Tensor] = None) -> None:
    a_ilv, o_ilv = isinstance(a, IlvPair), isinstance(out, IlvPair)
    if a_ilv:
        a, lda = (a.t, None), (lda if lda is not None else 2 * K)
    if o_ilv:
        out, ldob = (out.t, None), (ldob if ldob is not None else 2 * N)
    o_hi, o_lo = out if out is not None else (None, None)
    args = lib.GemmArgs(
        lib.ptr(a[0]), lib.ptr(a[1]), lib.ptr(w[0]), lib.ptr(w[1]), lib.ptr(bias), lib.ptr(residual),
        lib.ptr(out_f32), lib.ptr(o_hi), lib.ptr(o_lo), M, N, K,
        lda if lda is not None else K, ldw if ldw is not None else K,
        ldr if ldr is not None else N, ldo if ldo is not None else N, ldob if ldob is not None else N,
        act, precision, row_group, row_group_stride, row_group_off, res_row_mod)
    args.act_after_res = int(act_after_res)
    args.tile_policy = pipeline.tile_policy()
    args.pair_layout = lib.PAIR_A_ILV32 if a_ilv else lib.PAIR_SEPARATE
    args.out_pair_layout = lib.PAIR_A_ILV32 if o_ilv else lib.PAIR_SEPARATE
    if f16_col0:
        args.out_f16_col0 = int(f16_col0)
        splitk = 1
    if precision == lib.PREC_F16X2:
        splitk = 1
    if col_scale is not None:
        _chk(col_scale, torch.float32, "gemm.col_scale")
        splitk = 1
    if out_mask is not None:
        args.out_mask, args.ldm = lib.ptr(out_mask), ldm or N
    if residual_pair is not None:
        args.residual_hi, args.residual_lo = lib.ptr(residual_pair[0]), lib.ptr(residual_pair[1])
    S = 1
    plain = out_mask is None and not act_after_res and residual_pair is None
    if (a_ilv or o_ilv) and (not plain or splitk not in (None, 1)):
        raise lib.MvpError("interleaved pair operands: plain GEMMs only (no masks or split-K)")
    if plain and not a_ilv:
        S = splitk_auto(M, N, K) if splitk is None else int(splitk)
    if S > 1:
        ws = _splitk_workspace(M, N, S, a[0].device)
        args.splitk, args.splitk_ws, args.splitk_ws_bytes = S, lib.ptr(ws), ws.numel()
    tile = _route_label(M, N, K, precision, S, args.tile_policy, a_ilv, not plain) if (w_ilv is not None or _TRACE is not None) else ""
    if w_ilv is not None and tile.startswith("pp ") and ldw is None:
        args.w_hi, args.w_lo, args.ldw = lib.ptr(w_ilv), None, 2 * K
        args.pair_layout |= lib.PAIR_W_ILV32
    if col_scale is not None:
        name, args = "mvp_gemm_scaled", lib.GemmScaledArgs(args, lib.ptr(col_scale))
    else:
        name = "mvp_gemm_bias_act_res"
    _traced("gemm", tile, precision, 2.0 * M * N * K, lambda: lib.call(name, args))


def layernorm(x: torch.Tensor, gamma: torch.Tensor, beta: torch.Tensor, out: Optional[Pair], M: int, Cdim: int, eps: float,
              out_f32: Optional[torch.Tensor] = None, out_f16: bool = False) -> None:
    ilv = isinstance(out, IlvPair)
    if ilv:
        out = (out.t, None)
    elif out is None:
        out = (None, None)
    a = lib.LayerNormArgs(lib.ptr(x), lib.ptr(gamma), lib.ptr(beta), lib.ptr(out[0]), lib.ptr(out[1]), lib.ptr(out_f32), M, Cdim, eps,
                          lib.PAIR_A_ILV32 if ilv else lib.PAIR_SEPARATE, 1 if out_f16 else 0)
    nb = M * Cdim * (4 + (2 * (2 if (ilv or out[1] is not None) else 1) if (ilv or out[0] is not None) else 0) + (4 if out_f32 is not None else 0))
    _traced("hbm", "layernorm_kernel", 0, float(nb), lambda: lib.call("mvp_layernorm_fwd", a))


def attention(qkv: Pair, out: Pair, B: int, N: int, H: int, scale: float, precision: int, ld_qkv=None, ld_out=None, v_f16: bool = False,
              out_f16: bool = False, qk_f16: bool = False, bias: Optional[torch.Tensor] = None, ld_bias=None, bias_head_stride=None,
              rel: Optional[torch.Tensor] = None, rel_grid: Optional[Tuple[int, int]] = None) -> None:
    if qk_f16 and not v_f16:
        raise lib.MvpError("attention: qk_f16 needs v_f16 (mvp_attention_args.v_format = MVP_ATT_V_F16_QK_F16)")
    ilv = isinstance(out, IlvPair)
    if ilv:
        out, ld_out = (out.t, None), (ld_out if ld_out is not None else 2 * H * 64)
    a = lib.AttentionArgs(lib.ptr(qkv[0]), lib.ptr(qkv[1]), lib.ptr(out[0]), lib.ptr(out[1]), B, N, H,
                          ld_qkv if ld_qkv is not None else 3 * H * 64, ld_out if ld_out is not None else H * 64, scale, precision,
                          lib.PAIR_A_ILV32 if ilv else lib.PAIR_SEPARATE, (2 if qk_f16 else 1) if v_f16 else 0, 1 if out_f16 else 0)
    if rel is not None:
        if bias is not None:
            raise lib.MvpError("attention: a dense bias and decomposed relative-position terms exclude each other")
        if rel.dtype != torch.float32 or rel.dim() != 3 or rel.stride(2) != 1 or rel_grid is None:
            raise lib.MvpError("attention: rel must be fp32 [B * H, N, ld_rel] with unit column stride, with rel_grid=(Kh, Kw)")
        ar = lib.AttentionRelposArgs(a, lib.ptr(rel), rel.stride(0), rel.stride(1), int(rel_grid[0]), int(rel_grid[1]))
        _traced("attention", "4x32q relpos", precision, 4.0 * B * H * N * N * 64, lambda: lib.call("mvp_attention_relpos_fwd", ar))
        return
    if bias is not None:
        if bias.dtype != torch.float32 or bias.dim() != 3 or bias.stride(2) != 1:
            raise lib.MvpError("attention: bias must be fp32 [H, N, ld_bias] with unit column stride")
        ab = lib.AttentionBiasArgs(a, lib.ptr(bias), bias_head_stride if bias_head_stride is not None else bias.stride(0),
                                   ld_bias if ld_bias is not None else bias.stride(1))
        _traced("attention", "4x32q bias", precision, 4.0 * B * H * N * N * 64, lambda: lib.call("mvp_attention_bias_fwd", ab))
        return
    _traced("attention", "4x32q", precision, 4.0 * B * H * N * N * 64, lambda: lib.call("mvp_attention_fwd", a))


def rope2d_qkv(qkv_f32: torch.Tensor, out: Pair, cos_tab: torch.Tensor, sin_tab: torch.Tensor, M: int, N: int, H: int, n_prefix: int,
               gh: int, gw: int, precision: int, v_f16: bool = False, qk_f16: bool = False, ld_in=None, ld_out=None) -> None:
    if qk_f16 and not v_f16:
        raise lib.MvpError("rope2d_qkv: qk_f16 needs v_f16 (mvp_attention_args.v_format = MVP_ATT_V_F16_QK_F16)")
    _chk(cos_tab, torch.float32, "rope2d_qkv.cos_tab")
    _chk(sin_tab, torch.float32, "rope2d_qkv.sin_tab")
    if qkv_f32.dtype != torch.float32 or cos_tab.dim() != 2 or cos_tab.shape[1] != 32 or sin_tab.shape != cos_tab.shape:
        raise lib.MvpError("rope2d_qkv: fp32 projection and fp32 [rows, 32] cos / sin tables of one shape expected")
    a = lib.Rope2dQkvArgs(lib.ptr(qkv_f32), lib.ptr(out[0]), lib.ptr(out[1]), lib.ptr(cos_tab), lib.ptr(sin_tab), M, N, H, n_prefix, gh, gw,
                          int(cos_tab.shape[0]), ld_in if ld_in is not None else 3 * H * 64, ld_out if ld_out is not None else 3 * H * 64,
                          precision, (2 if qk_f16 else 1) if v_f16 else 0)
    nb = M * 3 * H * 64 * (4 + (4 if out[1] is not None else 2))
    _traced("hbm", "rope2d_qkv_kernel", 0, float(nb), lambda: lib.call("mvp_rope2d_qkv", a))


def relpos_terms(qkv_f32: torch.Tensor, out: Pair, rel: torch.Tensor, rh: torch.Tensor, rw: torch.Tensor, M: int, N: int, H: int, precision: int,
                 v_f16: bool = False, qk_f16: bool = False, ld_in=None, ld_out=None) -> None:
    if qk_f16 and not v_f16:
        raise lib.MvpError("relpos_terms: qk_f16 needs v_f16 (mvp_attention_args.v_format = MVP_ATT_V_F16_QK_F16)")
    _chk(rh, torch.float32, "relpos_terms.rh")
    _chk(rw, torch.float32, "relpos_terms.rw")
    if qkv_f32.dtype != torch.float32 or rh.dim() != 3 or rw.dim() != 3 or rh.shape[2] != 64 or rw.shape[2] != 64:
        raise lib.MvpError("relpos_terms: fp32 projection and fp32 [Q, K, 64] tables expected")
    if rel.dtype != torch.float32 or rel.dim() != 3 or rel.stride(2) != 1:
        raise lib.MvpError("relpos_terms: rel must be fp32 [B * H, N, ld_rel] with unit column stride")
    a = lib.RelposTermsArgs(lib.ptr(qkv_f32), lib.ptr(out[0]), lib.ptr(out[1]), lib.ptr(rel), lib.ptr(rh), lib.ptr(rw), rel.stride(0), M, N, H,
                            int(rh.shape[0]), int(rw.shape[0]), int(rh.shape[1]), int(rw.shape[1]),
                            ld_in if ld_in is not None else 3 * H * 64, ld_out if ld_out is not None else 3 * H * 64, rel.stride(1),
                            precision, (2 if qk_f16 else 1) if v_f16 else 0)
    nb = M * 3 * H * 64 * (4 + (4 if out[1] is not None else 2)) + M * H * (rh.shape[1] + rw.shape[1]) * 4
    _traced("hbm", "relpos_terms_kernel", 0, float(nb), lambda: lib.call("mvp_relpos_terms", a))


def gather_rows(src, dst, idx: torch.Tensor, rows_in: int, cols: int, ld_in=None, ld_out=None) -> None:
    if isinstance(src, IlvPair) != isinstance(dst, IlvPair):
        raise lib.MvpError("gather_rows: source and destination must have the same pair form")
    if isinstance(src, IlvPair):
        src, dst, cols = (src.t, None), (dst.t, None), 2 * cols
    if idx.dtype != torch.int32 or not idx.is_contiguous():
        raise lib.MvpError("gather_rows: idx must be a contiguous int32 tensor")
    a = lib.GatherRowsArgs(lib.ptr(src[0]), lib.ptr(src[1]), lib.ptr(dst[0]), lib.ptr(dst[1]), lib.ptr(idx), int(idx.numel()), int(rows_in), int(cols),
                           ld_in if ld_in is not None else cols, ld_out if ld_out is not None else cols)
    nb = idx.numel() * cols * 2 * (2 if src[1] is not None else 1) * 2
    _traced("hbm", "gather_rows_kernel", 0, float(nb), lambda: lib.call("mvp_gather_rows", a))


def cls_rows(cls: torch.Tensor, pos0: torch.Tensor, x: torch.Tensor, B: int, N: int, Cdim: int) -> None:
    lib.call("mvp_cls_rows", lib.ClsRowsArgs(lib.ptr(cls), lib.ptr(pos0), lib.ptr(x), B, N, Cdim))


def prefix_rows(cls: torch.Tensor, pos0: torch.Tensor, reg: Optional[torch.Tensor], x: torch.Tensor, B: int, N: int, Cdim: int) -> None:
    R = 0 if reg is None else int(reg.shape[0])
    lib.call("mvp_prefix_rows", lib.PrefixRowsArgs(lib.ptr(cls), lib.ptr(pos0), lib.ptr(reg), lib.ptr(x), B, N, Cdim, R))


def bn_tokens_workspace_bytes(M: int, Cdim: int) -> int:
    return int(lib.load().mvp_bn_tokens_workspace_bytes(M, Cdim))


def bn_tokens_to_nchw(x, B, N, Cdim, hw, *, workspace, stats=None, gamma=None, beta=None, running_mean=None, running_var=None,
                      nchw=None, tok: Optional[Pair] = None, ld_tok=0, col_off=0, tokT: Optional[Pair] = None, ldT=0,
                      eps=1e-5, momentum=0.1, mode=0, cls_out=None, num_batches_tracked=None, defer_running=False,
                      groups=1, stats_gstride=0, nchw_gstride=0, tok_gstride=0, cls_gstride=0) -> None:
    t_hi, t_lo = tok if tok is not None else (None, None)
    tt_hi, tt_lo = tokT if tokT is not None else (None, None)
    a = lib.BnTokensArgs(lib.ptr(x), lib.ptr(gamma), lib.ptr(beta), lib.ptr(running_mean), lib.ptr(running_var), lib.ptr(stats),
                         lib.ptr(nchw), lib.ptr(t_hi), lib.ptr(t_lo), ld_tok, col_off, lib.ptr(tt_hi), lib.ptr(tt_lo), ldT,
                         lib.ptr(workspace), workspace.numel() * workspace.element_size(), B, N, Cdim, hw, eps, momentum, mode, lib.ptr(cls_out),
                         lib.ptr(num_batches_tracked) if mode == 0 else None, int(bool(defer_running) and mode == 0),
                         int(groups), int(stats_gstride), int(nchw_gstride), int(tok_gstride), int(cls_gstride))
    M = B * N * max(1, int(groups))
    B = B * max(1, int(groups))
    nb = M * Cdim * 4 * (2 if mode == 0 else 1) + B * hw * Cdim * ((4 if nchw is not None else 0) + (4 if tok is not None and tok[1] is not None else (2 if tok is not None else 0)))
    _traced("hbm", "bn_tokens (partial+finalize+apply)", 0, float(nb), lambda: lib.call("mvp_bn_tokens_to_nchw_fwd", a))


def bn_running_update(stats, running_mean, running_var, num_batches_tracked, Cdim, momentum=0.1) -> None:
    lib.call("mvp_bn_running_update", lib.BnRunningUpdateArgs(lib.ptr(stats), lib.ptr(running_mean), lib.ptr(running_var),
                                                               lib.ptr(num_batches_tracked), Cdim, momentum))


def bn_running_update_many(items, momentum=0.1) -> None:
    if len({it[1].data_ptr() for it in items}) != len(items):
        for st, rm, rv, nbt, Cdim in items:
            bn_running_update(st, rm, rv, nbt, Cdim, momentum)
        return
    for i0 in range(0, len(items), lib.BN_RUNNING_MAX):
        part = items[i0:i0 + lib.BN_RUNNING_MAX]
        arr = (lib.BnRunningUpdateArgs * len(part))(*[
            lib.BnRunningUpdateArgs(lib.ptr(st), lib.ptr(rm), lib.ptr(rv), lib.ptr(nbt), Cdim, momentum) for st, rm, rv, nbt, Cdim in part])
        lib.check(lib.load().mvp_bn_running_update_n(arr, len(part), lib.stream_ptr()), "mvp_bn_running_update_n")


def pack_nchw_tokens(nchw: torch.Tensor, B: int, Cdim: int, hw: int, *, tok: Optional[Pair] = None, ld_tok=0, col_off=0,
                     tokT: Optional[Pair] = None, ldT=0) -> None:
    t_hi, t_lo = tok if tok is not None else (None, None)
    tt_hi, tt_lo = tokT if tokT is not None else (None, None)
    a = lib.PackNchwArgs(lib.ptr(nchw), lib.ptr(t_hi), lib.ptr(t_lo), ld_tok, col_off, lib.ptr(tt_hi), lib.ptr(tt_lo), ldT, B, Cdim, hw)
    lib.call("mvp_pack_nchw_tokens", a)


def resize(src: torch.Tensor, dst: torch.Tensor, planes: int, Hi: int, Wi: int, Ho: int, Wo: int, mode: int, *, align_corners=False,
           channels_last=False, Cdim=0, scale_h=0.0, scale_w=0.0, backward=False) -> None:
    a = lib.ResizeArgs(lib.ptr(src), lib.ptr(dst), planes, Hi, Wi, Ho, Wo, mode, int(align_corners), int(channels_last), Cdim, scale_h, scale_w)
    lib.call("mvp_resize_bwd" if backward else "mvp_resize_fwd", a)


def depth_predict_fwd(logits, depth, inv_sum, P, K, min_depth, max_depth, kind) -> None:
    a = lib.DepthPredictArgs(lib.ptr(logits), lib.ptr(depth), lib.ptr(inv_sum), None, None, P, K, min_depth, max_depth, kind)
    lib.call("mvp_depth_predict_fwd", a)


def depth_predict_bwd(logits, depth, inv_sum, grad_depth, grad_logits, P, K, min_depth, max_depth, kind) -> None:
    a = lib.DepthPredictArgs(lib.ptr(logits), lib.ptr(depth), lib.ptr(inv_sum), lib.ptr(grad_depth), lib.ptr(grad_logits), P, K, min_depth, max_depth, kind)
    lib.call("mvp_depth_predict_bwd", a)


def depth_loss_workspace_bytes(B: int, HW: int) -> int:
    return int(lib.load().mvp_depth_loss_workspace_bytes(B, HW))


def depth_loss(pred, target, loss, grad_pred, workspace, B, HW, w_sig=10.0, w_grad=0.5, max_depth=10.0, eps=1e-3, sigma=0.85) -> None:
    a = lib.DepthLossArgs(lib.ptr(pred), lib.ptr(target), lib.ptr(loss), lib.ptr(grad_pred), lib.ptr(workspace),
                          workspace.numel() * workspace.element_size(), B, HW, w_sig, w_grad, max_depth, eps, sigma)
    _traced("hbm", "depth_loss (dlf_stats+dlf_grad)" if B <= 16 else "depth_loss (dl_stats+dl_pairs+dl_finalize+dl_grad)", 0, float(B * HW * 12), lambda: lib.call("mvp_depth_loss_fwd_bwd", a))


def angular_loss(pred, gt, mask_u8, loss, grad_pred, workspace, B, Cp, HW, eps=1e-4) -> None:
    a = lib.AngularLossArgs(lib.ptr(pred), lib.ptr(gt), lib.ptr(mask_u8), lib.ptr(loss), lib.ptr(grad_pred), lib.ptr(workspace),
                            workspace.numel() * workspace.element_size(), B, Cp, HW, eps)
    lib.call("mvp_angular_loss_fwd_bwd", a)


def colsum(x, out, M, N, ld=None, accumulate=False, workspace=None) -> None:
    if workspace is None:
        workspace = torch.empty(int(lib.load().mvp_colsum_workspace_bytes(M, N)) // 4 + 4, dtype=torch.float32, device=x.device)
    lib.call("mvp_colsum", lib.ColsumArgs(lib.ptr(x), lib.ptr(out), M, N, ld if ld is not None else N, int(accumulate),
                                          lib.ptr(workspace), workspace.numel() * workspace.element_size()))


def adamw_step(param, grad, exp_avg, exp_avg_sq, hyper, n, beta1=0.9, beta2=0.999, eps=1e-8, weight_decay=0.01, grad_scale=1.0,
               lr=0.0, bias_c1=0.0, bias_c2=0.0) -> None:
    a = lib.AdamWArgs(lib.ptr(param), lib.ptr(grad), lib.ptr(exp_avg), lib.ptr(exp_avg_sq), lib.ptr(hyper), n, beta1, beta2, eps, weight_decay, grad_scale,
                      lr, bias_c1, bias_c2)
    lib.call("mvp_adamw_step", a)


def corr_argmax(src_feat, tgt_feat, kp_xy, out_xy, out_val, workspace, Cdim, h, w, K, heat_out=None) -> None:
    a = lib.CorrArgmaxArgs(lib.ptr(src_feat), lib.ptr(tgt_feat), lib.ptr(kp_xy), lib.ptr(out_xy), lib.ptr(out_val), lib.ptr(workspace),
                           workspace.numel() * workspace.element_size(), Cdim, h, w, K, lib.ptr(heat_out))
    lib.call("mvp_corr_argmax", a)


def knn_ratio(src_feat, tgt_feat, src_valid, tgt_valid, nn_idx, dist, weight, n_valid, workspace, Cdim, N0, N1) -> None:
    a = lib.KnnRatioArgs(lib.ptr(src_feat), lib.ptr(tgt_feat), lib.ptr(src_valid), lib.ptr(tgt_valid), lib.ptr(nn_idx), lib.ptr(dist),
                         lib.ptr(weight), lib.ptr(n_valid), lib.ptr(workspace), workspace.numel() * workspace.element_size(), Cdim, N0, N1)
    lib.call("mvp_knn_ratio", a)


def bn_act_workspace(device) -> torch.Tensor:
    return torch.empty(lib.BN_ACT_WORKSPACE_BYTES // 8, dtype=torch.float64, device=device)


def _bn_act_args(x, B, HW, Cdim, ld, act, training, *, y=None, gamma=None, beta=None, running_mean=None, running_var=None,
                 num_batches_tracked=None, stats=None, grad_y=None, grad_x=None, grad_gamma=None, grad_beta=None, workspace=None, n=0,
                 eps=1e-5, momentum=0.1, accumulate=False):
    return lib.BnActArgs(lib.ptr(x), lib.ptr(y), lib.ptr(gamma), lib.ptr(beta), lib.ptr(running_mean), lib.ptr(running_var),
                         lib.ptr(num_batches_tracked), lib.ptr(stats), lib.ptr(grad_y), lib.ptr(grad_x), lib.ptr(grad_gamma), lib.ptr(grad_beta),
                         lib.ptr(workspace), workspace.numel() * workspace.element_size() if workspace is not None else 0,
                         B, HW, Cdim, ld, int(n), eps, momentum, act, int(training), int(accumulate))


def bn_act_fwd(x, y, B, HW, Cdim, ld, act, training, **kw) -> None:
    a = _bn_act_args(x, B, HW, Cdim, ld, act, training, y=y, **kw)
    work = float(B * HW * Cdim * 4 * (3 if (act == lib.BN_ACT_SIGMOID and training) else 2))
    _traced("hbm", "bn_act_fwd", 0, work, lambda: lib.call("mvp_bn_act_fwd", a))


def bn_act_bwd(x, grad_y, grad_x, B, HW, Cdim, ld, act, training, **kw) -> None:
    a = _bn_act_args(x, B, HW, Cdim, ld, act, training, grad_y=grad_y, grad_x=grad_x, **kw)
    work = float(B * HW * 4 * ((4 if act == lib.BN_ACT_SIGMOID else 2) * Cdim + ld))
    _traced("hbm", "bn_act_bwd", 0, work, lambda: lib.call("mvp_bn_act_bwd", a))


def bce_loss(pred, target, loss, grad_pred, workspace, N) -> None:
    a = lib.BceLossArgs(lib.ptr(pred), lib.ptr(target), lib.ptr(loss), lib.ptr(grad_pred), lib.ptr(workspace),
                        workspace.numel() * workspace.element_size(), N)
    _traced("hbm", "bce_loss", 0, float(N * (12 if grad_pred is not None else 8)), lambda: lib.call("mvp_bce_loss_fwd_bwd", a))


def binary_counts(pred, gt, counts, G, n, threshold=0.5) -> None:
    a = lib.BinaryCountsArgs(lib.ptr(pred), lib.ptr(gt), lib.ptr(counts), G, n, threshold)
    _traced("hbm", "binary_counts", 0, float(G * n * 8), lambda: lib.call("mvp_binary_counts", a))
```

### midvision-probe_amd/mvp/optim.py

```python
from __future__ import annotations

from typing import Iterable, Optional

import torch

from . import ops


_GRAD_DST = {}


def grad_destination(param: torch.Tensor):
    ent = _GRAD_DST.get(id(param))
    if ent is None:
        return None
    flat, off, n, shape, ref = ent
    if ref() is not param:
        return None
    if param.grad is not None:
        return None
    return flat[off:off + n].view(shape)


class FlatAdamW(torch.optim.Optimizer):
    def __init__(self, params, lr=1e-3, betas=(0.9, 0.999), eps=1e-8, weight_decay=1e-2, process_group=None,
                 overlap_comm: bool = False, broadcast_init: bool = True, force_comm: bool = False):
        defaults = dict(lr=lr, betas=betas, eps=eps, weight_decay=weight_decay)
        super().__init__(params, defaults)
        if len(self.param_groups) != 1:
            raise NotImplementedError("FlatAdamW handles the single probe parameter group of the trainers (model_lr == 0)")
        plist = [p for p in self.param_groups[0]["params"] if p.requires_grad]
        if not plist:
            raise ValueError("no trainable parameters")
        dev = plist[0].device
        if dev.type != "cuda":
            raise RuntimeError("FlatAdamW needs device parameters (no CPU fallback)")
        sizes = [(p.numel() + 3) // 4 * 4 for p in plist]
        total = sum(sizes)
        self.flat_param = torch.zeros(total, dtype=torch.float32, device=dev)
        self.flat_grad = torch.zeros(total, dtype=torch.float32, device=dev)
        self.exp_avg = torch.zeros(total, dtype=torch.float32, device=dev)
        self.exp_avg_sq = torch.zeros(total, dtype=torch.float32, device=dev)
        off = 0
        with torch.no_grad():
            for p, sz in zip(plist, sizes):
                n = p.numel()
                self.flat_param[off:off + n].copy_(p.detach().reshape(-1))
                p.data = self.flat_param[off:off + n].view(p.shape)
                p.grad = self.flat_grad[off:off + n].view(p.shape)
                off += sz
        import weakref

        off = 0
        for p, sz in zip(plist, sizes):
            _GRAD_DST[id(p)] = (self.flat_grad, off, p.numel(), tuple(p.shape), weakref.ref(p))
            weakref.finalize(p, _GRAD_DST.pop, id(p), None)
            off += sz
        self._params = plist
        self._n = total
        self._step = 0
        self.process_group = process_group
        self.overlap_comm = bool(overlap_comm)
        import os

        self.force_comm = bool(force_comm) or os.environ.get("MVP_FORCE_COMM") == "1"
        self._pending = None
        self._comm_buf = None
        from .dist import world_size as _world

        if broadcast_init and _world(process_group) > 1:
            import torch.distributed as dist

            dist.broadcast(self.flat_param, src=dist.get_global_rank(process_group, 0) if process_group is not None else 0, group=process_group)

    def zero_grad(self, set_to_none: bool = True):
        for p in self._params:
            p.grad = None

    def _gather_stray_grads(self):
        off = 0
        for p in self._params:
            n = p.numel()
            want = self.flat_grad.data_ptr() + off * 4
            if p.grad is None:
                self.flat_grad[off:off + n].zero_()
                p.grad = self.flat_grad[off:off + n].view(p.shape)
            elif p.grad.data_ptr() != want:
                self.flat_grad[off:off + n].copy_(p.grad.reshape(-1))
                p.grad = self.flat_grad[off:off + n].view(p.shape)
            off += (n + 3) // 4 * 4

    def all_reduce_grads(self):
        from .dist import all_reduce_sum_flat

        return all_reduce_sum_flat(self.flat_grad, self.process_group)

    def _apply(self, grad: torch.Tensor, world: int, lr: float, step: int):
        g = self.param_groups[0]
        b1, b2 = g["betas"]
        ops.adamw_step(self.flat_param, grad, self.exp_avg, self.exp_avg_sq, None, self._n,
                       beta1=b1, beta2=b2, eps=g["eps"], weight_decay=g["weight_decay"], grad_scale=1.0 / world,
                       lr=lr, bias_c1=1.0 - b1 ** step, bias_c2=1.0 - b2 ** step)

    @torch.no_grad()
    def finish_pending(self):
        if self._pending is None:
            return
        work, world, lr, step = self._pending
        self._pending = None
        if work is not None:
            work.wait()
        self._apply(self._comm_buf, world, lr, step)

    @torch.no_grad()
    def step(self, closure=None):
        self.finish_pending()
        self._gather_stray_grads()
        return self._step_flat()

    def step_in_place(self):
        self.finish_pending()
        self._opt_called = True
        return self._step_flat()

    def _step_flat(self):
        self._step += 1
        lr = float(self.param_groups[0]["lr"])
        from .dist import world_size as _world

        world = _world(self.process_group)
        if self.overlap_comm and (world > 1 or (self.force_comm and torch.distributed.is_available() and torch.distributed.is_initialized())):
            import torch.distributed as dist

            if self._comm_buf is None:
                self._comm_buf = torch.empty_like(self.flat_grad)
            self._comm_buf.copy_(self.flat_grad)
            work = dist.all_reduce(self._comm_buf, op=dist.ReduceOp.SUM, group=self.process_group, async_op=True)
            self._pending = (work, world, lr, self._step)
            return None
        world = self.all_reduce_grads()
        self._apply(self.flat_grad, world, lr, self._step)
        return None

    def grad_slots(self):
        out, off = [], 0
        for p in self._params:
            n = p.numel()
            out.append((p, self.flat_grad[off:off + n].view(p.shape)))
            off += (n + 3) // 4 * 4
        return out

    def state_dict(self):
        self.finish_pending()
        return super().state_dict()
```

Baseline: 10800.

## Fuse probe weight pair split into AdamW and bins backward with bias colsum

Adds an AdamW variant that writes the hi/lo split pair of the probe weight directly while updating parameters, with a version-tracked cache so the next forward can reuse the pair without a separate split kernel. Adds a fused linear-bins backward that also emits the split gradient pair (with zero padding) and computes the bias gradient column sum via last-arriver atomic counters inside the same launch. The aim is fewer kernel launches and fewer passes over the probe gradient and weights. It adds cache invalidation logic and cross-block atomic synchronisation that must stay correct.

```diff
diff --git a/include/mvp_hip.h b/include/mvp_hip.h
--- a/include/mvp_hip.h
+++ b/include/mvp_hip.h
@@ -469,6 +469,25 @@
 int64_t mvp_gemm_tn_workspace_bytes(int Cout, int Cin, int kh, int kw, int splits);
 int mvp_gemm_tn_conv(const mvp_gemm_tn_args*, void* stream);
 
+typedef struct mvp_adamw_pair_args mvp_adamw_pair_args;
+struct mvp_adamw_pair_args {
+  mvp_adamw_args step;
+  mvp_bf16* pair_hi; mvp_bf16* pair_lo;
+  int64_t pair_off;
+  int rows, cols, ld;
+};
+int mvp_adamw_step_pair(const mvp_adamw_pair_args*, void* stream);
+
+typedef struct mvp_linear_bins_bwd_fused_args mvp_linear_bins_bwd_fused_args;
+struct mvp_linear_bins_bwd_fused_args {
+  mvp_linear_bins_args bins;
+  mvp_bf16* g_hi; mvp_bf16* g_lo; int ldg;
+  float* bias_grad;
+  void* workspace; int64_t workspace_bytes;
+};
+int64_t mvp_linear_bins_bwd_fused_workspace_bytes(int M, int K);
+int mvp_linear_bins_bwd_fused(const mvp_linear_bins_bwd_fused_args*, void* stream);
+
 #ifdef __cplusplus
 }
 #endif
diff --git a/midvision-probe_amd/csrc/colsum_order.h b/midvision-probe_amd/csrc/colsum_order.h
--- /dev/null
+++ b/midvision-probe_amd/csrc/colsum_order.h
@@ -0,0 +1,55 @@
+#pragma once
+#include "mvp_common.h"
+
+constexpr int CS_CHUNK = 64;
+
+__host__ __device__ inline int cs_chunk_rows(int M) {
+  const int r = (M + 255) / 256;
+  return r < CS_CHUNK ? CS_CHUNK : ((r + 3) & ~3);
+}
+
+__device__ __forceinline__ void colsum_partial_block(const float* x, int M, int N, int ld, float* part, int chunk, int cgroup, int ychunk,
+                                                     float (*red)[64]) {
+  const int c = cgroup * 64 + (threadIdx.x & 63);
+  const int rg = threadIdx.x >> 6;
+  const int r0 = ychunk * chunk, r1 = min(M, r0 + chunk);
+  float s = 0.f;
+  if (c < N) {
+    float s0 = 0.f, s1 = 0.f, s2 = 0.f, s3 = 0.f;
+    int r = r0 + rg;
+    for (; r + 12 < r1; r += 16) {
+      s0 += x[(size_t)r * ld + c];
+      s1 += x[(size_t)(r + 4) * ld + c];
+      s2 += x[(size_t)(r + 8) * ld + c];
+      s3 += x[(size_t)(r + 12) * ld + c];
+    }
+    for (; r < r1; r += 4) s0 += x[(size_t)r * ld + c];
+    s = (s0 + s1) + (s2 + s3);
+  }
+  red[rg][threadIdx.x & 63] = s;
+  __syncthreads();
+  if (rg == 0 && c < N)
+    part[(size_t)ychunk * N + c] = (red[0][threadIdx.x] + red[1][threadIdx.x]) + (red[2][threadIdx.x] + red[3][threadIdx.x]);
+}
+
+__device__ __forceinline__ void colsum_final_block(const float* part, int nchunk, int N, float* out, int accumulate, int cgroup, float (*red)[64]) {
+  const int lc = threadIdx.x & 63, rg = threadIdx.x >> 6;
+  const int c = cgroup * 64 + lc;
+  float s0 = 0.f, s1 = 0.f, s2 = 0.f, s3 = 0.f;
+  if (c < N) {
+    int k = rg;
+    for (; k + 12 < nchunk; k += 16) {
+      s0 += part[(size_t)k * N + c];
+      s1 += part[(size_t)(k + 4) * N + c];
+      s2 += part[(size_t)(k + 8) * N + c];
+      s3 += part[(size_t)(k + 12) * N + c];
+    }
+    for (; k < nchunk; k += 4) s0 += part[(size_t)k * N + c];
+  }
+  red[rg][lc] = (s0 + s1) + (s2 + s3);
+  __syncthreads();
+  if (rg == 0 && c < N) {
+    const float s = (red[0][lc] + red[1][lc]) + (red[2][lc] + red[3][lc]);
+    out[c] = accumulate ? out[c] + s : s;
+  }
+}
diff --git a/midvision-probe_amd/csrc/head.hip b/midvision-probe_amd/csrc/head.hip
--- a/midvision-probe_amd/csrc/head.hip
+++ b/midvision-probe_amd/csrc/head.hip
@@ -1,4 +1,5 @@
 #include "mvp_common.h"
+#include "colsum_order.h"
 
 namespace {
 
@@ -62,11 +63,35 @@
   }
 }
 
-__global__ __launch_bounds__(256) void linear_bins_bwd_kernel(const mvp_linear_bins_args p) {
-  const int lane = threadIdx.x & 63;
+struct BinsPairOut {
+  uint16_t* hi; uint16_t* lo; int ldg;
+};
+
+template <bool PAIR>
+__device__ __forceinline__ void bins_store_row4(const mvp_linear_bins_args& p, const BinsPairOut& q, int64_t tok, int k, const float4 o) {
+  *(float4*)(p.grad_l0 + tok * p.K + k) = o;
+  if (PAIR) {
+    uint16_t h[4], l[4];
+    split_bf16(o.x, h[0], l[0]); split_bf16(o.y, h[1], l[1]);
+    split_bf16(o.z, h[2], l[2]); split_bf16(o.w, h[3], l[3]);
+    *(u32x2_t*)(q.hi + tok * q.ldg + k) = u32x2_t{pack2(h[0], h[1]), pack2(h[2], h[3])};
+    if (q.lo) *(u32x2_t*)(q.lo + tok * q.ldg + k) = u32x2_t{pack2(l[0], l[1]), pack2(l[2], l[3])};
+  }
+}
+
+template <bool PAIR>
+__device__ __forceinline__ void bins_zero_pad(const mvp_linear_bins_args& p, const BinsPairOut& q, int64_t tok, int lane) {
+  if (PAIR) {
+    for (int k = p.K + lane * 4; k < q.ldg; k += 256) {
+      *(u32x2_t*)(q.hi + tok * q.ldg + k) = u32x2_t{0u, 0u};
+      if (q.lo) *(u32x2_t*)(q.lo + tok * q.ldg + k) = u32x2_t{0u, 0u};
+    }
+  }
+}
+
+template <bool PAIR>
+__device__ __forceinline__ void bins_bwd_generic_token(const mvp_linear_bins_args& p, const BinsPairOut& q, const int64_t tok, const int lane) {
   const int Ho = p.h * p.f, Wo = p.w * p.f;
-  const int64_t tok = (int64_t)blockIdx.x * 4 + (threadIdx.x >> 6);
-  if (tok >= (int64_t)p.B * p.h * p.w) return;
   const int tx = (int)(tok % p.w);
   const int64_t r = tok / p.w;
   const int ty = (int)(r % p.h);
@@ -109,8 +134,15 @@
     o.y = bin_value(k + 1, p.K, p.min_depth, p.max_depth) * s1[1] - s2[1];
     o.z = bin_value(k + 2, p.K, p.min_depth, p.max_depth) * s1[2] - s2[2];
     o.w = bin_value(k + 3, p.K, p.min_depth, p.max_depth) * s1[3] - s2[3];
-    *(float4*)(p.grad_l0 + tok * p.K + k) = o;
-  }
+    bins_store_row4<PAIR>(p, q, tok, k, o);
+  }
+  bins_zero_pad<PAIR>(p, q, tok, lane);
+}
+
+__global__ __launch_bounds__(256) void linear_bins_bwd_kernel(const mvp_linear_bins_args p) {
+  const int64_t tok = (int64_t)blockIdx.x * 4 + (threadIdx.x >> 6);
+  if (tok >= (int64_t)p.B * p.h * p.w) return;
+  bins_bwd_generic_token<false>(p, BinsPairOut{nullptr, nullptr, 0}, tok, threadIdx.x & 63);
 }
 
 
@@ -192,11 +224,9 @@
   }
 }
 
-__global__ __launch_bounds__(256) void linear_bins_bwd_fast(const mvp_linear_bins_args p) {
-  const int lane = threadIdx.x & 63;
+template <bool PAIR>
+__device__ __forceinline__ void bins_bwd_fast_token(const mvp_linear_bins_args& p, const BinsPairOut& q, const int64_t tok, const int lane) {
   const int Ho = p.h * p.f, Wo = p.w * p.f;
-  const int64_t tok = (int64_t)blockIdx.x * 4 + (threadIdx.x >> 6);
-  if (tok >= (int64_t)p.B * p.h * p.w) return;
   const int tx = (int)(tok % p.w);
   const int64_t r = tok / p.w;
   const int ty = (int)(r % p.h);
@@ -265,9 +295,98 @@
   o.y = bin_value(k + 1, 256, p.min_depth, p.max_depth) * s1[1] - s2[1];
   o.z = bin_value(k + 2, 256, p.min_depth, p.max_depth) * s1[2] - s2[2];
   o.w = bin_value(k + 3, 256, p.min_depth, p.max_depth) * s1[3] - s2[3];
-  *(float4*)(p.grad_l0 + tok * 256 + k) = o;
-}
-
+  bins_store_row4<PAIR>(p, q, tok, k, o);
+  bins_zero_pad<PAIR>(p, q, tok, lane);
+}
+
+__global__ __launch_bounds__(256) void linear_bins_bwd_fast(const mvp_linear_bins_args p) {
+  const int64_t tok = (int64_t)blockIdx.x * 4 + (threadIdx.x >> 6);
+  if (tok >= (int64_t)p.B * p.h * p.w) return;
+  bins_bwd_fast_token<false>(p, BinsPairOut{nullptr, nullptr, 0}, tok, threadIdx.x & 63);
+}
+
+constexpr int BINS_CTR_ALIGN = 256;
+
+__host__ __device__ inline int64_t bins_ctr_bytes(int nchunk) {
+  return ((int64_t)(nchunk + 1) * 4 + BINS_CTR_ALIGN - 1) / BINS_CTR_ALIGN * BINS_CTR_ALIGN;
+}
+
+__device__ __forceinline__ bool last_arriver(int* ctr, int expect, int* s_flag) {
+  asm volatile("s_waitcnt vmcnt(0)" ::: "memory");
+  __syncthreads();
+  if (threadIdx.x == 0) {
+    __builtin_amdgcn_fence(__ATOMIC_RELEASE, "agent");
+    asm volatile("s_waitcnt vmcnt(0)" ::: "memory");
+    *s_flag = (__hip_atomic_fetch_add(ctr, 1, __ATOMIC_RELAXED, __HIP_MEMORY_SCOPE_AGENT) == expect - 1) ? 1 : 0;
+  }
+  __syncthreads();
+  if (!*s_flag) return false;
+  if (threadIdx.x == 0) {
+    __builtin_amdgcn_fence(__ATOMIC_ACQUIRE, "agent");
+    __hip_atomic_store(ctr, 0, __ATOMIC_RELAXED, __HIP_MEMORY_SCOPE_AGENT);
+  }
+  asm volatile("s_waitcnt vmcnt(0)" ::: "memory");
+  __syncthreads();
+  return true;
+}
+
+template <bool FAST>
+__global__ __launch_bounds__(256) void linear_bins_bwd_fused_kernel(const mvp_linear_bins_bwd_fused_args a, const int chunk, const int nchunk) {
+  __shared__ float red[4][64];
+  __shared__ int s_flag;
+  const mvp_linear_bins_args& p = a.bins;
+  const int T = p.B * p.h * p.w;
+  const BinsPairOut q{(uint16_t*)a.g_hi, (uint16_t*)a.g_lo, a.ldg};
+  const int64_t tok = (int64_t)blockIdx.x * 4 + (threadIdx.x >> 6);
+  if (tok < T) {
+    if (FAST) bins_bwd_fast_token<true>(p, q, tok, threadIdx.x & 63);
+    else bins_bwd_generic_token<true>(p, q, tok, threadIdx.x & 63);
+  }
+  if (!a.bias_grad) return;
+  int* ctr = (int*)a.workspace;
+  float* part = (float*)((char*)a.workspace + bins_ctr_bytes(nchunk));
+  const int ch = (int)(((int64_t)blockIdx.x * 4) / chunk);
+  const int rows = min(T, (ch + 1) * chunk) - ch * chunk;
+  if (!last_arriver(ctr + ch, (rows + 3) >> 2, &s_flag)) return;
+  const int groups = (p.K + 63) >> 6;
+  for (int cg = 0; cg < groups; ++cg) {
+    colsum_partial_block(p.grad_l0, T, p.K, p.K, part, chunk, cg, ch, red);
+    __syncthreads();
+  }
+  if (!last_arriver(ctr + nchunk, nchunk, &s_flag)) return;
+  for (int cg = 0; cg < groups; ++cg) {
+    colsum_final_block(part, nchunk, p.K, a.bias_grad, 0, cg, red);
+    __syncthreads();
+  }
+}
+
+}
+
+extern "C" int64_t mvp_linear_bins_bwd_fused_workspace_bytes(int M, int K) {
+  if (M <= 0 || K <= 0) return 0;
+  const int chunk = cs_chunk_rows(M);
+  const int nchunk = (M + chunk - 1) / chunk;
+  return bins_ctr_bytes(nchunk) + (int64_t)nchunk * K * 4;
+}
+
+extern "C" int mvp_linear_bins_bwd_fused(const mvp_linear_bins_bwd_fused_args* f, void* stream) {
+  if (!f) return MVP_EINVAL;
+  const mvp_linear_bins_args* a = &f->bins;
+  if (!a->grad_depth || !a->grad_l0 || !a->depth || !a->inv_sum || !a->gate || !f->g_hi) return MVP_EINVAL;
+  if (a->B <= 0 || a->h <= 0 || a->w <= 0 || a->f < 1 || a->K < 8 || (a->K & 7)) return MVP_EINVAL;
+  if (f->ldg < a->K || (f->ldg & 7) || (((uintptr_t)f->g_hi | (uintptr_t)f->g_lo) & 7)) return MVP_EINVAL;
+  const int64_t T = (int64_t)a->B * a->h * a->w;
+  if (T * a->f * a->f >= ((int64_t)1 << 31)) return MVP_EINVAL;
+  const int chunk = cs_chunk_rows((int)T);
+  const int nchunk = (int)((T + chunk - 1) / chunk);
+  if (f->bias_grad && (!f->workspace || ((uintptr_t)f->workspace & 15) || f->workspace_bytes < mvp_linear_bins_bwd_fused_workspace_bytes((int)T, a->K)))
+    return MVP_EINVAL;
+  if (a->K == 256 && a->f <= 4)
+    hipLaunchKernelGGL(linear_bins_bwd_fused_kernel<true>, dim3((unsigned)((T + 3) / 4)), dim3(256), 0, (hipStream_t)stream, *f, chunk, nchunk);
+  else
+    hipLaunchKernelGGL(linear_bins_bwd_fused_kernel<false>, dim3((unsigned)((T + 3) / 4)), dim3(256), 0, (hipStream_t)stream, *f, chunk, nchunk);
+  MVP_LAUNCH_CHECK();
+  return MVP_OK;
 }
 
 extern "C" int mvp_linear_bins_fwd(const mvp_linear_bins_args* a, void* stream) {
diff --git a/midvision-probe_amd/csrc/info.hip b/midvision-probe_amd/csrc/info.hip
--- a/midvision-probe_amd/csrc/info.hip
+++ b/midvision-probe_amd/csrc/info.hip
@@ -32,6 +32,7 @@
   MVP_SZ(mvp_gemm_scaled_args) MVP_SZ(mvp_patch_gather_ld_args) MVP_SZ(mvp_prefix_rows_args) MVP_SZ(mvp_gemm_route_t) MVP_SZ(mvp_rope2d_qkv_args) MVP_SZ(mvp_attention_bias_args)
   MVP_SZ(mvp_gather_rows_args) MVP_SZ(mvp_relpos_terms_args) MVP_SZ(mvp_attention_relpos_args) MVP_SZ(mvp_knn_ratio_args)
   MVP_SZ(mvp_bn_act_args) MVP_SZ(mvp_bce_loss_args) MVP_SZ(mvp_binary_counts_args)
+  MVP_SZ(mvp_adamw_pair_args) MVP_SZ(mvp_linear_bins_bwd_fused_args)
 #undef MVP_SZ
   return -1;
 }
diff --git a/midvision-probe_amd/csrc/optim.hip b/midvision-probe_amd/csrc/optim.hip
--- a/midvision-probe_amd/csrc/optim.hip
+++ b/midvision-probe_amd/csrc/optim.hip
@@ -2,7 +2,14 @@
 
 namespace {
 
-__global__ __launch_bounds__(256) void adamw_kernel(const mvp_adamw_args p) {
+struct AdamWPairOut {
+  uint16_t* hi; uint16_t* lo;
+  int64_t off, count;
+  int cols, ld;
+};
+
+template <bool PAIR>
+__device__ __forceinline__ void adamw_body(const mvp_adamw_args& p, const AdamWPairOut& q) {
   const float lr = p.hyper ? p.hyper[0] : p.lr, bc1 = p.hyper ? p.hyper[1] : p.bias_c1, bc2 = p.hyper ? p.hyper[2] : p.bias_c2;
   const float step_size = lr / bc1;
   const float rbc2 = 1.0f / sqrtf(bc2);
@@ -25,6 +32,18 @@
     ((float4*)p.param)[i] = w;
     ((float4*)p.exp_avg)[i] = m;
     ((float4*)p.exp_avg_sq)[i] = v;
+    if (PAIR) {
+      const int64_t e = (i << 2) - q.off;
+      if (e >= 0 && e < q.count) {
+        const int64_t r = e / q.cols;
+        const int64_t o = r * q.ld + (e - r * q.cols);
+        uint16_t h[4], l[4];
+        split_bf16(wp[0], h[0], l[0]); split_bf16(wp[1], h[1], l[1]);
+        split_bf16(wp[2], h[2], l[2]); split_bf16(wp[3], h[3], l[3]);
+        *(u32x2_t*)(q.hi + o) = u32x2_t{pack2(h[0], h[1]), pack2(h[2], h[3])};
+        if (q.lo) *(u32x2_t*)(q.lo + o) = u32x2_t{pack2(l[0], l[1]), pack2(l[2], l[3])};
+      }
+    }
   }
   if (blockIdx.x == 0 && threadIdx.x < (p.n & 3)) {
     const int64_t i = (n4 << 2) + threadIdx.x;
@@ -37,16 +56,42 @@
   }
 }
 
+__global__ __launch_bounds__(256) void adamw_kernel(const mvp_adamw_args p) {
+  adamw_body<false>(p, AdamWPairOut{nullptr, nullptr, 0, 0, 1, 1});
+}
+
+__global__ __launch_bounds__(256) void adamw_pair_kernel(const mvp_adamw_pair_args a) {
+  adamw_body<true>(a.step, AdamWPairOut{(uint16_t*)a.pair_hi, (uint16_t*)a.pair_lo, a.pair_off, (int64_t)a.rows * a.cols, a.cols, a.ld});
+}
+
+int adamw_check(const mvp_adamw_args* a) {
+  if (!a->param || !a->grad || !a->exp_avg || !a->exp_avg_sq || a->n <= 0) return MVP_EINVAL;
+  if (!a->hyper && !(a->bias_c1 > 0.f && a->bias_c2 > 0.f)) return MVP_EINVAL;
+  if (((uintptr_t)a->param | (uintptr_t)a->grad | (uintptr_t)a->exp_avg | (uintptr_t)a->exp_avg_sq) & 15) return MVP_EINVAL;
+  return MVP_OK;
+}
+
+unsigned adamw_grid(int64_t n) {
+  int64_t g = ((n >> 2) + 255) / 256;
+  if (g < 1) g = 1;
+  if (g > 2048) g = 2048;
+  return (unsigned)g;
+}
+
+}
+
+extern "C" int mvp_adamw_step_pair(const mvp_adamw_pair_args* a, void* stream) {
+  if (!a || adamw_check(&a->step) != MVP_OK || !a->pair_hi) return MVP_EINVAL;
+  if (a->pair_off < 0 || (a->pair_off & 3) || a->rows <= 0 || a->cols <= 0 || (a->cols & 3) || (a->ld & 3) || a->ld < a->cols) return MVP_EINVAL;
+  if (a->pair_off + (int64_t)a->rows * a->cols > a->step.n || (((uintptr_t)a->pair_hi | (uintptr_t)a->pair_lo) & 7)) return MVP_EINVAL;
+  hipLaunchKernelGGL(adamw_pair_kernel, dim3(adamw_grid(a->step.n)), dim3(256), 0, (hipStream_t)stream, *a);
+  MVP_LAUNCH_CHECK();
+  return MVP_OK;
 }
 
 extern "C" int mvp_adamw_step(const mvp_adamw_args* a, void* stream) {
-  if (!a || !a->param || !a->grad || !a->exp_avg || !a->exp_avg_sq || a->n <= 0) return MVP_EINVAL;
-  if (!a->hyper && !(a->bias_c1 > 0.f && a->bias_c2 > 0.f)) return MVP_EINVAL;
-  if (((uintptr_t)a->param | (uintptr_t)a->grad | (uintptr_t)a->exp_avg | (uintptr_t)a->exp_avg_sq) & 15) return MVP_EINVAL;
-  int64_t g = ((a->n >> 2) + 255) / 256;
-  if (g < 1) g = 1;
-  if (g > 2048) g = 2048;
-  hipLaunchKernelGGL(adamw_kernel, dim3((unsigned)g), dim3(256), 0, (hipStream_t)stream, *a);
+  if (!a || adamw_check(a) != MVP_OK) return MVP_EINVAL;
+  hipLaunchKernelGGL(adamw_kernel, dim3(adamw_grid(a->n)), dim3(256), 0, (hipStream_t)stream, *a);
   MVP_LAUNCH_CHECK();
   return MVP_OK;
 }
diff --git a/midvision-probe_amd/csrc/probe.hip b/midvision-probe_amd/csrc/probe.hip
--- a/midvision-probe_amd/csrc/probe.hip
+++ b/midvision-probe_amd/csrc/probe.hip
@@ -1,4 +1,5 @@
 #include "mvp_common.h"
+#include "colsum_order.h"
 
 namespace {
 
@@ -62,58 +63,14 @@
   }
 }
 
-constexpr int CS_CHUNK = 64;
-
-__host__ __device__ inline int cs_chunk_rows(int M) {
-  const int r = (M + 255) / 256;
-  return r < CS_CHUNK ? CS_CHUNK : ((r + 3) & ~3);
-}
-
 __global__ __launch_bounds__(256) void colsum_partial_kernel(const mvp_colsum_args p, float* part, int chunk) {
   __shared__ float red[4][64];
-  const int c = blockIdx.x * 64 + (threadIdx.x & 63);
-  const int rg = threadIdx.x >> 6;
-  const int r0 = blockIdx.y * chunk, r1 = min(p.M, r0 + chunk);
-  float s = 0.f;
-  if (c < p.N) {
-    float s0 = 0.f, s1 = 0.f, s2 = 0.f, s3 = 0.f;
-    int r = r0 + rg;
-    for (; r + 12 < r1; r += 16) {
-      s0 += p.x[(size_t)r * p.ld + c];
-      s1 += p.x[(size_t)(r + 4) * p.ld + c];
-      s2 += p.x[(size_t)(r + 8) * p.ld + c];
-      s3 += p.x[(size_t)(r + 12) * p.ld + c];
-    }
-    for (; r < r1; r += 4) s0 += p.x[(size_t)r * p.ld + c];
-    s = (s0 + s1) + (s2 + s3);
-  }
-  red[rg][threadIdx.x & 63] = s;
-  __syncthreads();
-  if (rg == 0 && c < p.N)
-    part[(size_t)blockIdx.y * p.N + c] = (red[0][threadIdx.x] + red[1][threadIdx.x]) + (red[2][threadIdx.x] + red[3][threadIdx.x]);
+  colsum_partial_block(p.x, p.M, p.N, p.ld, part, chunk, blockIdx.x, blockIdx.y, red);
 }
 
 __global__ __launch_bounds__(256) void colsum_final_kernel(const mvp_colsum_args p, const float* part, int nchunk) {
   __shared__ float red[4][64];
-  const int lc = threadIdx.x & 63, rg = threadIdx.x >> 6;
-  const int c = blockIdx.x * 64 + lc;
-  float s0 = 0.f, s1 = 0.f, s2 = 0.f, s3 = 0.f;
-  if (c < p.N) {
-    int k = rg;
-    for (; k + 12 < nchunk; k += 16) {
-      s0 += part[(size_t)k * p.N + c];
-      s1 += part[(size_t)(k + 4) * p.N + c];
-      s2 += part[(size_t)(k + 8) * p.N + c];
-      s3 += part[(size_t)(k + 12) * p.N + c];
-    }
-    for (; k < nchunk; k += 4) s0 += part[(size_t)k * p.N + c];
-  }
-  red[rg][lc] = (s0 + s1) + (s2 + s3);
-  __syncthreads();
-  if (rg == 0 && c < p.N) {
-    const float s = (red[0][lc] + red[1][lc]) + (red[2][lc] + red[3][lc]);
-    p.out[c] = p.accumulate ? p.out[c] + s : s;
-  }
+  colsum_final_block(part, nchunk, p.N, p.out, p.accumulate, blockIdx.x, red);
 }
 
 inline int grid_for(int64_t work) {
diff --git a/midvision-probe_amd/mvp/functional.py b/midvision-probe_amd/mvp/functional.py
--- a/midvision-probe_amd/mvp/functional.py
+++ b/midvision-probe_amd/mvp/functional.py
@@ -90,14 +90,17 @@
 
 
 def _head_weight_grad(gl0: torch.Tensor, K: int, pack: PackedFeatures, pr: int, dst: Optional[torch.Tensor] = None) -> torch.Tensor:
-    from . import conv
-    dev = gl0.device
     Kg = (K + 127) // 128 * 128
     if Kg != K:
         gpad = gl0.new_zeros(pack.M, Kg)
         gpad[:, :K] = gl0
         gl0 = gpad
-    gp = ops.split_bf16(gl0, pr)
+    return _head_weight_grad_pair(ops.split_bf16(gl0, pr), Kg, K, pack, pr, dst)
+
+
+def _head_weight_grad_pair(gp, Kg: int, K: int, pack: PackedFeatures, pr: int, dst: Optional[torch.Tensor] = None) -> torch.Tensor:
+    from . import conv
+    dev = gp[0].device
     dW = dst if (dst is not None and pack.Cpad == pack.Ctot and tuple(dst.shape) == (K, pack.Cpad)) else torch.empty(K, pack.Cpad, dtype=torch.float32, device=dev)
     geo = dict(B=pack.B, H=pack.h, W=pack.w, C=pack.Cpad, Ho=pack.h, Wo=pack.w, kh=1, kw=1, stride=1, pad=0, up=0)
     conv.conv_dw(gp, Kg, pack.tok, pack.Cpad, geo, K, dW, precision=pr)
@@ -154,12 +157,18 @@
 def linear_bins_forward(weight, bias, pack: PackedFeatures, precision: int, min_depth: float, max_depth: float):
     K, Ctot = weight.shape[0], pack.Ctot
     dev = weight.device
-    w2 = weight.detach().reshape(K, Ctot).float()
-    if pack.Cpad != Ctot:
-        wpad = w2.new_zeros(K, pack.Cpad)
-        wpad[:, :Ctot] = w2
-        w2 = wpad
-    wp = ops.split_bf16(w2.contiguous(), precision)
+    wp = None
+    if ops.probe_fused():
+        from .optim import weight_pair
+
+        wp = weight_pair(weight, K, Ctot, pack.Cpad, precision)
+    if wp is None:
+        w2 = weight.detach().reshape(K, Ctot).float()
+        if pack.Cpad != Ctot:
+            wpad = w2.new_zeros(K, pack.Cpad)
+            wpad[:, :Ctot] = w2
+            w2 = wpad
+        wp = ops.split_bf16(w2.contiguous(), precision)
     l0 = torch.empty(pack.M, K, dtype=torch.float32, device=dev)
     ops.gemm(pack.tok, wp, pack.M, K, pack.Cpad, bias=bias.detach().float().contiguous(), out_f32=l0, precision=precision)
     B, h, w = pack.B, pack.h, pack.w
@@ -177,8 +186,15 @@
     B, h, w = pack.B, pack.h, pack.w
     dev = gd.device
     gl0 = torch.empty(pack.M, K, dtype=torch.float32, device=dev)
-    a = lib.LinearBinsArgs(None, lib.ptr(depth), lib.ptr(inv), lib.ptr(gate), lib.ptr(gd.contiguous().float()), lib.ptr(gl0), B, h, w, K, 4,
+    gd = gd.contiguous().float()
+    a = lib.LinearBinsArgs(None, lib.ptr(depth), lib.ptr(inv), lib.ptr(gate), lib.ptr(gd), lib.ptr(gl0), B, h, w, K, 4,
                            min_depth, max_depth)
+    if ops.probe_fused() and pack.M * 16 < 2 ** 31:
+        Kg = (K + 127) // 128 * 128
+        gp = ops.empty_pair((pack.M, Kg), precision, dev)
+        db = db_dst if db_dst is not None else torch.empty(K, dtype=torch.float32, device=dev)
+        ops.linear_bins_bwd_fused(a, gp, Kg, db, pack.M, K)
+        return _head_weight_grad_pair(gp, Kg, K, pack, precision, dst=dw_dst), db
     lib.call("mvp_linear_bins_bwd", a)
     dW = _head_weight_grad(gl0, K, pack, precision, dst=dw_dst)
     db = db_dst
diff --git a/midvision-probe_amd/mvp/lib.py b/midvision-probe_amd/mvp/lib.py
--- a/midvision-probe_amd/mvp/lib.py
+++ b/midvision-probe_amd/mvp/lib.py
@@ -255,6 +255,14 @@
     _fields_ = [("g_hi", _vp), ("g_lo", _vp), ("x_hi", _vp), ("x_lo", _vp), ("partial", _vp), ("dw", _vp), ("zero_page", _vp),
                 ("M", _i64), ("Cout", _i), ("Cin", _i), ("ldg", _i), ("ldx", _i), ("H", _i), ("W", _i), ("Ho", _i), ("Wo", _i),
                 ("kh", _i), ("kw", _i), ("stride", _i), ("pad", _i), ("up", _i), ("splits", _i), ("accumulate", _i), ("precision", _i)]
+
+
+class AdamWPairArgs(C.Structure):
+    _fields_ = [("step", AdamWArgs), ("pair_hi", _vp), ("pair_lo", _vp), ("pair_off", _i64), ("rows", _i), ("cols", _i), ("ld", _i)]
+
+
+class LinearBinsBwdFusedArgs(C.Structure):
+    _fields_ = [("bins", LinearBinsArgs), ("g_hi", _vp), ("g_lo", _vp), ("ldg", _i), ("bias_grad", _vp), ("workspace", _vp), ("workspace_bytes", _i64)]
 
 
 SYMBOLS = {
@@ -321,6 +329,9 @@
     "mvp_bn_act_bwd": BnActArgs,
     "mvp_bce_loss_fwd_bwd": BceLossArgs,
     "mvp_binary_counts": BinaryCountsArgs,
+    "mvp_adamw_step_pair": AdamWPairArgs,
+    "mvp_linear_bins_bwd_fused_workspace_bytes": None,
+    "mvp_linear_bins_bwd_fused": LinearBinsBwdFusedArgs,
 }
 
 NEW_STRUCTS_ABI7 = {"mvp_gemm_scaled_args": GemmScaledArgs, "mvp_patch_gather_ld_args": PatchGatherLdArgs, "mvp_prefix_rows_args": PrefixRowsArgs}
@@ -329,7 +340,8 @@
                     "mvp_gather_rows_args": GatherRowsArgs, "mvp_relpos_terms_args": RelposTermsArgs,
                     "mvp_attention_relpos_args": AttentionRelposArgs, "mvp_knn_ratio_args": KnnRatioArgs,
                     "mvp_bn_act_args": BnActArgs, "mvp_bce_loss_args": BceLossArgs,
-                    "mvp_binary_counts_args": BinaryCountsArgs}
+                    "mvp_binary_counts_args": BinaryCountsArgs, "mvp_adamw_pair_args": AdamWPairArgs,
+                    "mvp_linear_bins_bwd_fused_args": LinearBinsBwdFusedArgs}
 
 _lib: Optional[C.CDLL] = None
 
@@ -377,6 +389,8 @@
     lib.mvp_gemm_tn_workspace_bytes.restype = _i64
     lib.mvp_depth_loss_workspace_bytes.argtypes = [_i, _i64]
     lib.mvp_depth_loss_workspace_bytes.restype = _i64
+    lib.mvp_linear_bins_bwd_fused_workspace_bytes.argtypes = [_i, _i]
+    lib.mvp_linear_bins_bwd_fused_workspace_bytes.restype = _i64
     _lib = lib
     return lib
 
diff --git a/midvision-probe_amd/mvp/ops.py b/midvision-probe_amd/mvp/ops.py
--- a/midvision-probe_amd/mvp/ops.py
+++ b/midvision-probe_amd/mvp/ops.py
@@ -2,6 +2,7 @@
 
 import ctypes
 import functools
+import os
 from typing import Optional, Tuple
 
 import torch
@@ -396,10 +397,40 @@
 
 
 def adamw_step(param, grad, exp_avg, exp_avg_sq, hyper, n, beta1=0.9, beta2=0.999, eps=1e-8, weight_decay=0.01, grad_scale=1.0,
-               lr=0.0, bias_c1=0.0, bias_c2=0.0) -> None:
+               lr=0.0, bias_c1=0.0, bias_c2=0.0, pair: Optional[Pair] = None, pair_off: int = 0, pair_rows: int = 0, pair_cols: int = 0) -> None:
     a = lib.AdamWArgs(lib.ptr(param), lib.ptr(grad), lib.ptr(exp_avg), lib.ptr(exp_avg_sq), lib.ptr(hyper), n, beta1, beta2, eps, weight_decay, grad_scale,
                       lr, bias_c1, bias_c2)
-    lib.call("mvp_adamw_step", a)
+    if pair is None:
+        lib.call("mvp_adamw_step", a)
+        return
+    lib.call("mvp_adamw_step_pair", lib.AdamWPairArgs(a, lib.ptr(pair[0]), lib.ptr(pair[1]), int(pair_off), int(pair_rows), int(pair_cols),
+                                                      int(pair[0].shape[-1])))
+
+
+def probe_fused() -> bool:
+    return os.environ.get("MVP_PROBE_FUSED", "1") != "0"
+
+
+_BINS_WS = {}
+
+
+def bins_bwd_workspace_bytes(M: int, K: int) -> int:
+    return int(lib.load().mvp_linear_bins_bwd_fused_workspace_bytes(M, K))
+
+
+def _bins_bwd_workspace(M: int, K: int, device) -> torch.Tensor:
+    need = bins_bwd_workspace_bytes(M, K)
+    key = _ws_key(device)
+    ws = _BINS_WS.get(key)
+    if ws is None or ws.numel() < need:
+        ws = _BINS_WS[key] = torch.zeros(max(need, 1 << 20), dtype=torch.uint8, device=device)
+    return ws
+
+
+def linear_bins_bwd_fused(bins_args, g_pair: Pair, ldg: int, bias_grad: torch.Tensor, M: int, K: int) -> None:
+    ws = _bins_bwd_workspace(M, K, bias_grad.device)
+    lib.call("mvp_linear_bins_bwd_fused", lib.LinearBinsBwdFusedArgs(bins_args, lib.ptr(g_pair[0]), lib.ptr(g_pair[1]), int(ldg), lib.ptr(bias_grad),
+                                                                      lib.ptr(ws), ws.numel()))
 
 
 def corr_argmax(src_feat, tgt_feat, kp_xy, out_xy, out_val, workspace, Cdim, h, w, K, heat_out=None) -> None:
diff --git a/midvision-probe_amd/mvp/optim.py b/midvision-probe_amd/mvp/optim.py
--- a/midvision-probe_amd/mvp/optim.py
+++ b/midvision-probe_amd/mvp/optim.py
@@ -20,6 +20,36 @@
     if param.grad is not None:
         return None
     return flat[off:off + n].view(shape)
+
+
+_PAIR_OWNER = {}
+
+
+def pair_spec_ok(numel: int, rows: int, cols: int, ld: int) -> bool:
+    return rows > 0 and cols > 0 and rows * cols == numel and cols % 4 == 0 and ld % 4 == 0 and ld >= cols
+
+
+class OperandPair:
+
+    def __init__(self, param_id: int, off: int, rows: int, cols: int, ld: int, precision: int, pair):
+        self.spec = (param_id, rows, cols, ld, precision)
+        self.off, self.rows, self.cols, self.ld, self.pair = off, rows, cols, ld, pair
+        self.versions = None
+
+    def written(self, versions) -> None:
+        self.versions = tuple(versions)
+
+    def invalidate(self) -> None:
+        self.versions = None
+
+    def current(self, versions) -> bool:
+        return self.versions is not None and self.versions == tuple(versions)
+
+
+def weight_pair(param: torch.Tensor, rows: int, cols: int, ld: int, precision: int):
+    ref = _PAIR_OWNER.get(id(param))
+    opt = ref() if ref is not None else None
+    return opt.operand_pair(param, rows, cols, ld, precision) if opt is not None else None
 
 
 class FlatAdamW(torch.optim.Optimizer):
@@ -55,7 +85,10 @@
         for p, sz in zip(plist, sizes):
             _GRAD_DST[id(p)] = (self.flat_grad, off, p.numel(), tuple(p.shape), weakref.ref(p))
             weakref.finalize(p, _GRAD_DST.pop, id(p), None)
+            _PAIR_OWNER[id(p)] = weakref.ref(self)
+            weakref.finalize(p, _PAIR_OWNER.pop, id(p), None)
             off += sz
+        self._pair: Optional[OperandPair] = None
         self._params = plist
         self._n = total
         self._step = 0
@@ -98,9 +131,48 @@
     def _apply(self, grad: torch.Tensor, world: int, lr: float, step: int):
         g = self.param_groups[0]
         b1, b2 = g["betas"]
+        kw = {}
+        slot = self._pair
+        if slot is not None:
+            p = self._pair_param()
+            if p is not None and ops.probe_fused():
+                kw = dict(pair=slot.pair, pair_off=slot.off, pair_rows=slot.rows, pair_cols=slot.cols)
+            else:
+                slot.invalidate()
         ops.adamw_step(self.flat_param, grad, self.exp_avg, self.exp_avg_sq, None, self._n,
                        beta1=b1, beta2=b2, eps=g["eps"], weight_decay=g["weight_decay"], grad_scale=1.0 / world,
-                       lr=lr, bias_c1=1.0 - b1 ** step, bias_c2=1.0 - b2 ** step)
+                       lr=lr, bias_c1=1.0 - b1 ** step, bias_c2=1.0 - b2 ** step, **kw)
+        if kw:
+            slot.written((p._version, self.flat_param._version))
+
+    def _pair_param(self):
+        slot = self._pair
+        for p, off in self._offsets():
+            if id(p) == slot.spec[0]:
+                return p if (off == slot.off and p.data_ptr() == self.flat_param.data_ptr() + off * 4) else None
+        return None
+
+    def _offsets(self):
+        off = 0
+        for p in self._params:
+            yield p, off
+            off += (p.numel() + 3) // 4 * 4
+
+    def invalidate_operand_pair(self) -> None:
+        if self._pair is not None:
+            self._pair.invalidate()
+
+    def operand_pair(self, param, rows: int, cols: int, ld: int, precision: int):
+        slot = self._pair
+        if slot is None or slot.spec != (id(param), rows, cols, ld, precision):
+            self._pair = None
+            for p, off in self._offsets():
+                if p is param and p.dtype == torch.float32 and pair_spec_ok(p.numel(), rows, cols, ld):
+                    self._pair = OperandPair(id(p), off, rows, cols, ld, precision, ops.zeros_pair((rows, ld), precision, p.device))
+            return None
+        if self._pending is not None or self._pair_param() is not param:
+            return None
+        return slot.pair if slot.current((param._version, self.flat_param._version)) else None
 
     @torch.no_grad()
     def finish_pending(self):
```

Result: slower. 10680 (-1.1%).
